# latticeboltzmann/2d-lb

Hardware: AMD Instinct MI355X
Metric: MLUPS (million lattice updates per second), fused D2Q9 BGK step (higher is better)
Workload: dtype f32

## Files before the change

2d-lb_amd/csrc/kernels_deep.h:

```cpp
#pragma once

#ifdef LB_DIAG
#define LB_DEEP_NOCOLLIDE if (!(a.diag & 1))
#else
#define LB_DEEP_NOCOLLIDE
#endif

namespace {

constexpr int DEEP_RW = 1, DEEP_PFD = 1;
constexpr int DEEP_WSLOTS = 8;
constexpr bool deep_pairs(bool mask, int bc) { return !mask && bc == LB_BC_PERIODIC; }

template <int RW, int NL>
struct DeepState {
    Window w[RW > 0 ? RW : 1];
    f4a d0[NL];
    unsigned mhist;
};
typedef unsigned u4v __attribute__((ext_vector_type(4)));
struct DeepCtx {
    int lane, x4, ym, n_iter;
    bool store_lane;
    f4a (*mine)[64], (*other)[64];
    f4a (*ho)[64];
    f4a (*dma)[64];
    unsigned dma_off;
};
constexpr int DEEP_WHOLE = 0, DEEP_FRONT = 1, DEEP_BACK = 2;
constexpr int DEEP_HO_SLOTS = 10;

__device__ __forceinline__ void deep_window_load(f4a (*W)[64], int lane, int it, f4a d0, Window &w)
{
    const int gs = 2 + 3 * (it & 1);
    w.d0 = d0; w.d1 = W[0][lane]; w.d3 = W[1][lane];
    w.g2 = W[gs][lane]; w.g5 = W[gs + 1][lane]; w.g6 = W[gs + 2][lane];
}
template <bool DOWN>
__device__ __forceinline__ void deep_window_push(f4a (*W)[64], int lane, int it, f4a &d0, const f4a (&q)[9])
{
    typedef Dir<DOWN> D_;
    const int gs = 2 + 3 * (it & 1);
    d0 = q[0]; W[0][lane] = q[1]; W[1][lane] = q[3];
    W[gs][lane] = q[D_::A]; W[gs + 1][lane] = q[D_::B]; W[gs + 2][lane] = q[D_::C];
}
template <bool DOWN>
__device__ __forceinline__ void deep_publish(f4a (*W)[64], int lane, int gs, const f4a (&q)[9])
{
    typedef Dir<DOWN> D_;
    W[gs][lane] = q[D_::An]; W[gs + 1][lane] = q[D_::Bn]; W[gs + 2][lane] = q[D_::Cn];
}

constexpr int DEEP_NUM_RECORDS = -1;
__device__ __forceinline__ float *deep_uniform(const float *p)
{
    const unsigned long long v = (unsigned long long)p;
    const unsigned lo = __builtin_amdgcn_readfirstlane((unsigned)v), hi = __builtin_amdgcn_readfirstlane((unsigned)(v >> 32));
    return reinterpret_cast<float *>(((unsigned long long)hi << 32) | lo);
}
__device__ __forceinline__ f4a deep_buf_load(__amdgpu_buffer_rsrc_t r, int vo, int so, int imm)
{
    return __builtin_bit_cast(f4a, __builtin_amdgcn_raw_buffer_load_b128(r, vo + imm, so, 0));
}
template <int BC, bool MASK>
__device__ __forceinline__ void deep_row_load(const StepArgs &a, int r, int x4, Row1 &o)
{
    int ym, yp;
    o.have = step1_rows(a, r, o.rr, ym, yp);
    o.mk = uc4{0, 0, 0, 0};
    o.hsolid = false;
    o.hxc = -1;
    if (o.have) {
        const long long P = a.pitch, S = a.plane;
        const float *s = a.src;
        const int yl = o.rr;
        o.wp = WrapPatch{0.f, 0.f, 0.f, 0.f, 0.f, 0.f};
        if (BC == LB_BC_PERIODIC) {
            const int c = a.nx - 1 - x4;
            const bool wrap_w = x4 == 0, wrap_e = c >= 0 && c < 4;
            if (wrap_w) {
                o.wp.p1 = s[1 * S + (long long)yl * P + a.nx - 1];
                o.wp.p5 = s[5 * S + (long long)ym * P + a.nx - 1];
                o.wp.p8 = s[8 * S + (long long)yp * P + a.nx - 1];
            }
            if (wrap_e) {
                o.wp.w3 = s[3 * S + (long long)yl * P];
                o.wp.w6 = s[6 * S + (long long)ym * P];
                o.wp.w7 = s[7 * S + (long long)yp * P];
            }
        }
        const __amdgpu_buffer_rsrc_t r0 = __builtin_amdgcn_make_buffer_rsrc(deep_uniform(s + (long long)yl * P - 1), 0, DEEP_NUM_RECORDS, 0x00020000);
        const __amdgpu_buffer_rsrc_t rm = __builtin_amdgcn_make_buffer_rsrc(deep_uniform(s + (long long)ym * P - 1), 0, DEEP_NUM_RECORDS, 0x00020000);
        const __amdgpu_buffer_rsrc_t rp = __builtin_amdgcn_make_buffer_rsrc(deep_uniform(s + (long long)yp * P - 1), 0, DEEP_NUM_RECORDS, 0x00020000);
        const unsigned S4 = (unsigned)a.plane * 4u;
        const int vo = x4 * 4;
        o.q[0] = deep_buf_load(r0, vo, 0, 4);
        o.q[1] = deep_buf_load(r0, vo, (int)(S4), 0);
        o.q[2] = deep_buf_load(rm, vo, (int)(2u * S4), 4);
        o.q[3] = deep_buf_load(r0, vo, (int)(3u * S4), 8);
        o.q[4] = deep_buf_load(rp, vo, (int)(4u * S4), 4);
        o.q[5] = deep_buf_load(rm, vo, (int)(5u * S4), 0);
        o.q[6] = deep_buf_load(rm, vo, (int)(6u * S4), 8);
        o.q[7] = deep_buf_load(rp, vo, (int)(7u * S4), 8);
        o.q[8] = deep_buf_load(rp, vo, (int)(8u * S4), 0);
        if (MASK) o.mk = *reinterpret_cast<const uc4 *>(lane_ptr(a.mask + (long long)yl * a.fpitch, x4));
    } else {
        o.wp = WrapPatch{0.f, 0.f, 0.f, 0.f, 0.f, 0.f};
#pragma unroll
        for (int k = 0; k < 9; ++k) o.q[k] = f4a{0.f, 0.f, 0.f, 0.f};
    }
}
#ifdef LB_DIAG
constexpr bool DEEP_MANUAL = false;
#else
constexpr bool DEEP_MANUAL = true;
#endif
__device__ __forceinline__ u4v deep_rsrc_words(const float *p)
{
    const unsigned long long v = (unsigned long long)p;
    return u4v{(unsigned)__builtin_amdgcn_readfirstlane((unsigned)v), (unsigned)__builtin_amdgcn_readfirstlane((unsigned)(v >> 32)), (unsigned)DEEP_NUM_RECORDS,
               0x00020000u};
}
template <int BC, bool MASK>
__device__ __forceinline__ void deep_row_issue(const StepArgs &a, int r, int x4, Row1 &o)
{
    int ym, yp;
    o.have = step1_rows(a, r, o.rr, ym, yp);
    o.hsolid = false;
    o.hxc = -1;
    if (o.have) {
        const long long P = a.pitch, S = a.plane;
        const float *s = a.src;
        const int yl = o.rr;
        if (BC == LB_BC_PERIODIC) {
            const int c = a.nx - 1 - x4;
            const bool wrap_w = x4 == 0, wrap_e = c >= 0 && c < 4;
            if (wrap_w) {
                const float *e = s + a.nx - 1;
                asm volatile("global_load_dword a36, %0, off\n\tglobal_load_dword a37, %1, off\n\tglobal_load_dword a38, %2, off"
                             :: "v"(e + 1 * S + (long long)yl * P), "v"(e + 5 * S + (long long)ym * P), "v"(e + 8 * S + (long long)yp * P)
                             : "memory", "a36", "a37", "a38");
            }
            if (wrap_e) {
                asm volatile("global_load_dword a39, %0, off\n\tglobal_load_dword a40, %1, off\n\tglobal_load_dword a41, %2, off"
                             :: "v"(s + 3 * S + (long long)yl * P), "v"(s + 6 * S + (long long)ym * P), "v"(s + 7 * S + (long long)yp * P)
                             : "memory", "a39", "a40", "a41");
            }
        }
        const u4v r0 = deep_rsrc_words(s + (long long)yl * P - 1), rm = deep_rsrc_words(s + (long long)ym * P - 1),
                  rp = deep_rsrc_words(s + (long long)yp * P - 1);
        const unsigned S4 = (unsigned)a.plane * 4u;
        asm volatile("buffer_load_dwordx4 a[0:3], %0, %1, 0 offen offset:4\n\t"
                     "buffer_load_dwordx4 a[4:7], %0, %1, %4 offen\n\t"
                     "buffer_load_dwordx4 a[8:11], %0, %2, %5 offen offset:4\n\t"
                     "buffer_load_dwordx4 a[12:15], %0, %1, %6 offen offset:8\n\t"
                     "buffer_load_dwordx4 a[16:19], %0, %3, %7 offen offset:4\n\t"
                     "buffer_load_dwordx4 a[20:23], %0, %2, %8 offen\n\t"
                     "buffer_load_dwordx4 a[24:27], %0, %2, %9 offen offset:8\n\t"
                     "buffer_load_dwordx4 a[28:31], %0, %3, %10 offen offset:8\n\t"
                     "buffer_load_dwordx4 a[32:35], %0, %3, %11 offen"
                     :: "v"(x4 * 4), "s"(r0), "s"(rm), "s"(rp), "s"(S4), "s"(2u * S4), "s"(3u * S4), "s"(4u * S4), "s"(5u * S4), "s"(6u * S4),
                        "s"(7u * S4), "s"(8u * S4)
                     : "memory", "a0", "a1", "a2", "a3", "a4", "a5", "a6", "a7", "a8", "a9", "a10", "a11", "a12", "a13",
                       "a14", "a15", "a16", "a17", "a18", "a19", "a20", "a21", "a22", "a23", "a24", "a25", "a26", "a27", "a28",
                       "a29", "a30", "a31", "a32", "a33", "a34", "a35");
        if (MASK) asm volatile("global_load_dword a42, %0, off" :: "v"(lane_ptr(a.mask + (long long)yl * a.fpitch, x4)) : "memory", "a42");
    }
}
template <int BC, bool MASK, int N>
__device__ __forceinline__ void deep_row_take(Row1 &o)
{
    static_assert(N == 0 || N == 9 || N == 12, "the stores of one steady iteration, or nothing");
#define LB_DEEP_TAKE_OUTS "={a[0:3]}"(o.q[0]), "={a[4:7]}"(o.q[1]), "={a[8:11]}"(o.q[2]), "={a[12:15]}"(o.q[3]), \
                          "={a[16:19]}"(o.q[4]), "={a[20:23]}"(o.q[5]), "={a[24:27]}"(o.q[6]), "={a[28:31]}"(o.q[7]), "={a[32:35]}"(o.q[8])
    if (N == 0) asm volatile("s_waitcnt vmcnt(0)" : LB_DEEP_TAKE_OUTS :: "memory");
    else if (N == 9) asm volatile("s_waitcnt vmcnt(9)" : LB_DEEP_TAKE_OUTS :: "memory");
    else asm volatile("s_waitcnt vmcnt(12)" : LB_DEEP_TAKE_OUTS :: "memory");
#undef LB_DEEP_TAKE_OUTS
    o.wp = WrapPatch{0.f, 0.f, 0.f, 0.f, 0.f, 0.f};
    if (BC == LB_BC_PERIODIC)
        asm volatile("" : "={a36}"(o.wp.p1), "={a37}"(o.wp.p5), "={a38}"(o.wp.p8), "={a39}"(o.wp.w3), "={a40}"(o.wp.w6), "={a41}"(o.wp.w7));
    o.mk = uc4{0, 0, 0, 0};
    if (MASK) {
        unsigned m;
        asm volatile("" : "={a42}"(m));
        o.mk = __builtin_bit_cast(uc4, m);
    }
    if (!o.have) {
#pragma unroll
        for (int k = 0; k < 9; ++k) o.q[k] = f4a{0.f, 0.f, 0.f, 0.f};
        o.mk = uc4{0, 0, 0, 0};
    }
}

template <int BC, bool MASK>
__device__ __forceinline__ void deep_row_issue_lds(const StepArgs &a, int r, int x4, unsigned slot, Row1 &o)
{
    int ym, yp;
    o.have = step1_rows(a, r, o.rr, ym, yp);
    o.hsolid = false;
    o.hxc = -1;
    if (o.have) {
        const long long P = a.pitch, S = a.plane;
        const float *s = a.src;
        const int yl = o.rr;
        unsigned m0_kept;
        asm volatile("s_waitcnt lgkmcnt(0)" ::: "memory");
        if (BC == LB_BC_PERIODIC) {
            const int c = a.nx - 1 - x4;
            const bool wrap_w = x4 == 0, wrap_e = c >= 0 && c < 4;
            if (wrap_w) {
                const float *e = s + a.nx - 1;
                asm volatile("s_mov_b32 %0, m0\n\ts_mov_b32 m0, %4\n\ts_nop 0\n\tglobal_load_lds_dword %1, off\n\t"
                             "s_add_u32 m0, m0, 0x100\n\ts_nop 0\n\tglobal_load_lds_dword %2, off\n\t"
                             "s_add_u32 m0, m0, 0x100\n\ts_nop 0\n\tglobal_load_lds_dword %3, off\n\ts_mov_b32 m0, %0"
                             : "=&s"(m0_kept)
                             : "v"(e + 1 * S + (long long)yl * P), "v"(e + 5 * S + (long long)ym * P), "v"(e + 8 * S + (long long)yp * P),
                               "s"(slot + 9 * 1024 + 256)
                             : "memory", "scc");
            }
            if (wrap_e) {
                asm volatile("s_mov_b32 %0, m0\n\ts_mov_b32 m0, %4\n\ts_nop 0\n\tglobal_load_lds_dword %1, off\n\t"
                             "s_add_u32 m0, m0, 0x100\n\ts_nop 0\n\tglobal_load_lds_dword %2, off\n\t"
                             "s_add_u32 m0, m0, 0x100\n\ts_nop 0\n\tglobal_load_lds_dword %3, off\n\ts_mov_b32 m0, %0"
                             : "=&s"(m0_kept)
                             : "v"(s + 3 * S + (long long)yl * P), "v"(s + 6 * S + (long long)ym * P), "v"(s + 7 * S + (long long)yp * P),
                               "s"(slot + 9 * 1024 + 256)
                             : "memory", "scc");
            }
        }
        const u4v r0 = deep_rsrc_words(s + (long long)yl * P - 1), rm = deep_rsrc_words(s + (long long)ym * P - 1),
                  rp = deep_rsrc_words(s + (long long)yp * P - 1);
        const unsigned S4 = (unsigned)a.plane * 4u;
        const int v0 = x4 * 4, v4 = v0 + 4, v8 = v0 + 8;
        asm volatile("s_mov_b32 %0, m0\n\ts_mov_b32 m0, %15\n\ts_nop 0\n\tbuffer_load_dwordx4 %2, %4, 0 offen lds\n\t"
                     "s_add_u32 m0, m0, 0x400\n\ts_nop 0\n\tbuffer_load_dwordx4 %1, %4, %7 offen lds\n\t"
                     "s_add_u32 m0, m0, 0x400\n\ts_nop 0\n\tbuffer_load_dwordx4 %2, %5, %8 offen lds\n\t"
                     "s_add_u32 m0, m0, 0x400\n\ts_nop 0\n\tbuffer_load_dwordx4 %3, %4, %9 offen lds\n\t"
                     "s_add_u32 m0, m0, 0x400\n\ts_nop 0\n\tbuffer_load_dwordx4 %2, %6, %10 offen lds\n\t"
                     "s_add_u32 m0, m0, 0x400\n\ts_nop 0\n\tbuffer_load_dwordx4 %1, %5, %11 offen lds\n\t"
                     "s_add_u32 m0, m0, 0x400\n\ts_nop 0\n\tbuffer_load_dwordx4 %3, %5, %12 offen lds\n\t"
                     "s_add_u32 m0, m0, 0x400\n\ts_nop 0\n\tbuffer_load_dwordx4 %3, %6, %13 offen lds\n\t"
                     "s_add_u32 m0, m0, 0x400\n\ts_nop 0\n\tbuffer_load_dwordx4 %1, %6, %14 offen lds\n\ts_mov_b32 m0, %0"
                     : "=&s"(m0_kept)
                     : "v"(v0), "v"(v4), "v"(v8), "s"(r0), "s"(rm), "s"(rp), "s"(S4), "s"(2u * S4), "s"(3u * S4), "s"(4u * S4), "s"(5u * S4),
                       "s"(6u * S4), "s"(7u * S4), "s"(8u * S4), "s"(slot)
                     : "memory", "scc");
        if (MASK)
            asm volatile("s_mov_b32 %0, m0\n\ts_mov_b32 m0, %2\n\ts_nop 0\n\tglobal_load_lds_dword %1, off\n\ts_mov_b32 m0, %0"
                         : "=&s"(m0_kept) : "v"(lane_ptr(a.mask + (long long)yl * a.fpitch, x4)), "s"(slot + 9 * 1024) : "memory");
    }
}
template <int BC, bool MASK>
__device__ __forceinline__ void deep_row_take_lds(const f4a (*S)[64], int lane, Row1 &o)
{
    asm volatile("s_waitcnt vmcnt(0)" ::: "memory");
    if (o.have) {
#pragma unroll
        for (int k = 0; k < 9; ++k) o.q[k] = S[k][lane];
        const unsigned *X = reinterpret_cast<const unsigned *>(S[9]);
        o.mk = MASK ? __builtin_bit_cast(uc4, X[lane]) : uc4{0, 0, 0, 0};
        o.wp = WrapPatch{0.f, 0.f, 0.f, 0.f, 0.f, 0.f};
        if (BC == LB_BC_PERIODIC) {
            const float e1 = __builtin_bit_cast(float, X[64 + lane]), e2 = __builtin_bit_cast(float, X[128 + lane]),
                        e3 = __builtin_bit_cast(float, X[192 + lane]);
            o.wp = WrapPatch{e1, e2, e3, e1, e2, e3};
        }
    } else {
        o.wp = WrapPatch{0.f, 0.f, 0.f, 0.f, 0.f, 0.f};
#pragma unroll
        for (int k = 0; k < 9; ++k) o.q[k] = f4a{0.f, 0.f, 0.f, 0.f};
        o.mk = uc4{0, 0, 0, 0};
    }
}

__device__ __forceinline__ void deep_row_store(const StepArgs &a, int r, int x4, const f4a (&t)[9])
{
    const __amdgpu_buffer_rsrc_t rd = __builtin_amdgcn_make_buffer_rsrc(deep_uniform(a.dst + (long long)r * a.pitch), 0, DEEP_NUM_RECORDS, 0x00020000);
    const unsigned S4 = (unsigned)a.plane * 4u;
    const int vo = x4 * 4;
    asm volatile("" ::: "memory");
    if (a.nts != 0) {
#pragma unroll
        for (int k = 0; k < 9; ++k) __builtin_amdgcn_raw_buffer_store_b128(__builtin_bit_cast(u4v, t[k]), rd, vo, (int)(k * S4), 2);
    } else {
#pragma unroll
        for (int k = 0; k < 9; ++k) __builtin_amdgcn_raw_buffer_store_b128(__builtin_bit_cast(u4v, t[k]), rd, vo, (int)(k * S4), 0);
    }
}

template <int BC, bool MASK, bool MACRO, int D, int RW, bool DOWN, int NST, int S, int ROLE = DEEP_WHOLE>
__device__ __forceinline__ void deep_stage(const StepArgs &a, const DeepCtx &cx, const int i, const int it,
                                           DeepState<RW, D - 1 - RW> &st, f4a (&qin)[9], f4a &r4, f4a &u4, f4a &v4)
{
    if constexpr (S <= D) {
        constexpr int K = S - 1;
        const int lane = cx.lane, x4 = cx.x4;
        constexpr int L = K > RW ? K - RW - 1 : 0;
        f4a (*W)[64] = cx.mine + L * DEEP_WSLOTS;
        if constexpr (NST >= S) {
            int r, t0_, t1_;
            (void)step1_rows(a, DOWN ? cx.ym - 1 - (i - K) : cx.ym + (i - K), r, t0_, t1_);
            f4a t[9];
            if constexpr (K <= RW) {
                skirt_gather<DOWN>(st.w[K - 1], qin, t);
                window_push_dir<DOWN>(st.w[K - 1], qin);
            } else {
                Window w;
                deep_window_load(W, lane, it, st.d0[L], w);
                skirt_gather<DOWN>(w, qin, t);
                deep_window_push<DOWN>(W, lane, it, st.d0[L], qin);
            }
            LB_DEEP_NOCOLLIDE collide_row<BC, MASK, true>(a, x4, a.y0 + r, t, mask_bits(st.mhist, K), r4, u4, v4);
            if constexpr (S == D && ROLE == DEEP_FRONT) {
#pragma unroll
                for (int k = 0; k < 9; ++k) cx.ho[k][lane] = t[k];
                if (MASK) reinterpret_cast<unsigned *>(cx.ho[9])[lane] = __builtin_bit_cast(unsigned, mask_bits(st.mhist, K));
            } else if constexpr (S == D) {
#ifdef LB_DIAG
                if (!(a.diag & (1 << 22)))
#endif
                if (cx.store_lane) {
                    deep_row_store(a, r, x4, t);
                    if (MACRO) {
                        const long long m = (long long)r * a.fpitch;
                        store_moments(a, m, x4, r4, u4, v4);
                    }
                }
            } else {
                if constexpr (NST == S) {
                    if constexpr (S <= RW) deep_publish<DOWN>(cx.other + (D - 2 - RW) * DEEP_WSLOTS, lane, S == 1 ? 5 : 2, t);
                    else deep_publish<DOWN>(cx.other + (S - RW - 1) * DEEP_WSLOTS, lane, 2 + 3 * (S & 1), t);
                }
                deep_stage<BC, MASK, MACRO, D, RW, DOWN, NST, S + 1, ROLE>(a, cx, i, it, st, t, r4, u4, v4);
            }
        } else if constexpr (NST == S - 1) {
            if constexpr (K <= RW) window_push_dir<DOWN>(st.w[K - 1], qin);
            else deep_window_push<DOWN>(W, lane, it, st.d0[L], qin);
        }
    }
}

template <int BC, bool MASK, bool MACRO, int D, int RW, int PFD, bool DOWN, int NST, int PAR = -1, int ROLE = DEEP_WHOLE>
__device__ __forceinline__ void deep_iter(const StepArgs &a, const DeepCtx &cx, const int i_, DeepState<RW, D - 1 - RW> &st, Row1 &cur,
                                          Row1 &nxt)
{
    static_assert(RW >= 0 && RW <= 2 && D - 1 - RW >= 1 && (ROLE == DEEP_WHOLE ? D - 2 > RW : D - 2 >= RW),
                  "register windows hand over through the last LDS window while it is idle");
    static_assert((D - 1 - RW) * DEEP_WSLOTS <= 40, "a wave has 40 KB of LDS at four waves per CU");
    const int lane = cx.lane, x4 = cx.x4;
    const int i = NST < D ? NST - 1 : i_;
    const int it = PAR >= 0 ? PAR : i;
    auto row_at = [&](int p) { return DOWN ? cx.ym - 1 - p : cx.ym + p; };
    f4a (*MB)[64] = cx.mine + (D - 2 - RW) * DEEP_WSLOTS;
    if (RW >= 1 && NST == 2) { st.w[0].g2 = MB[5][lane]; st.w[0].g5 = MB[6][lane]; st.w[0].g6 = MB[7][lane]; }
    if (RW >= 2 && NST == 3) { st.w[RW >= 2 ? 1 : 0].g2 = MB[2][lane]; st.w[RW >= 2 ? 1 : 0].g5 = MB[3][lane]; st.w[RW >= 2 ? 1 : 0].g6 = MB[4][lane]; }
#ifdef LB_DIAG
    if (!((a.diag & (1 << 23)) && i > 0))
#endif
    if constexpr (ROLE != DEEP_BACK) {
        if (ROLE == DEEP_FRONT) {
            deep_row_take_lds<BC, MASK>(cx.dma, lane, cur);
            deep_row_issue_lds<BC, MASK>(a, row_at(min(i + 1, cx.n_iter - 1)), x4, cx.dma_off, nxt);
        } else if (PFD && DEEP_MANUAL) {
            deep_row_take<BC, MASK, (NST < D ? 0 : (MACRO ? 12 : 9))>(cur);
            deep_row_issue<BC, MASK>(a, row_at(min(i + 1, cx.n_iter - 1)), x4, nxt);
        } else {
            static_assert(PFD == 1 || ROLE == DEEP_BACK, "a march that gathers its rows gathers them one ahead");
            deep_row_load<BC, MASK>(a, row_at(min(i + 1, cx.n_iter - 1)), x4, nxt);
        }
    }
    f4a (&q1)[9] = cur.q;
    f4a r4, u4, v4;
    const uc4 mk = cur.mk;
    if (ROLE != DEEP_BACK && cur.have) {
        gather_merge<BC, true>(a, x4, q1, cur.wp);
        LB_DEEP_NOCOLLIDE collide_row<BC, MASK, true>(a, x4, a.y0 + cur.rr, q1, mk, r4, u4, v4);
    }
    if (NST == 1) {
        if constexpr (RW >= 1) deep_publish<DOWN>(cx.other + (D - 2 - RW) * DEEP_WSLOTS, lane, 5, q1);
        else deep_publish<DOWN>(cx.other, lane, 2 + 3 * 1, q1);
    }
    deep_stage<BC, MASK, MACRO, D, RW, DOWN, NST, 2, ROLE>(a, cx, i, it, st, q1, r4, u4, v4);
    if (MASK) st.mhist = ((st.mhist | mask_word(mk)) << 1) & (0x01010101u * (unsigned)(((1 << D) - 2) & 0xff));
    if (ROLE == DEEP_WHOLE && NST < D) __syncthreads();
}

template <int BC, bool MASK, bool MACRO, int D, int RW, int PFD, bool DOWN, int NST>
__device__ __forceinline__ void deep_fill(const StepArgs &a, const DeepCtx &cx, DeepState<RW, D - 1 - RW> &st, Row1 &ra, Row1 &rb)
{
    if constexpr (NST < D) {
        if ((NST & 1) == 0) deep_iter<BC, MASK, MACRO, D, RW, PFD, DOWN, NST>(a, cx, NST - 1, st, rb, ra);
        else deep_iter<BC, MASK, MACRO, D, RW, PFD, DOWN, NST>(a, cx, NST - 1, st, ra, rb);
        deep_fill<BC, MASK, MACRO, D, RW, PFD, DOWN, NST + 1>(a, cx, st, ra, rb);
    }
}

template <int BC, bool MASK, bool MACRO, int D, int RW, int PFD, bool DOWN>
__device__ __forceinline__ void deep_march(const StepArgs &a, const int x0, const int ym, const int len, f4a (*mine)[64],
                                           f4a (*other)[64])
{
    DeepCtx cx;
    cx.lane = threadIdx.x;
    const int xr = x0 + cx.lane * 4;
    cx.x4 = skirt_column<BC>(a, xr, deep_skirt_lanes(D));
    cx.store_lane = skirt_store_lane(a, cx.lane, xr, deep_skirt_lanes(D));
    cx.ym = ym; cx.n_iter = len + D - 1;
    cx.mine = mine; cx.other = other;
    DeepState<RW, D - 1 - RW> st = {};
    auto row_at = [&](int p) { return DOWN ? ym - 1 - p : ym + p; };
    static_assert(PFD == 1, "a whole march gathers one row ahead");
    Row1 ra, rb;
    if (DEEP_MANUAL) deep_row_issue<BC, MASK>(a, row_at(0), cx.x4, ra);
    else deep_row_load<BC, MASK>(a, row_at(0), cx.x4, ra);
    deep_fill<BC, MASK, MACRO, D, RW, PFD, DOWN, 1>(a, cx, st, ra, rb);
    if (DEEP_MANUAL) asm volatile("s_waitcnt vmcnt(0)" ::: "memory");
    if (!deep_pairs(MASK, BC)) {
        if ((D - 1) & 1) ra = rb;
        for (int i = D - 1; i < cx.n_iter; ++i) {
            deep_iter<BC, MASK, MACRO, D, RW, PFD, DOWN, D>(a, cx, i, st, ra, rb);
            ra = rb;
        }
    } else {
        constexpr int P0 = (D - 1) & 1;
        int i = D - 1;
        for (; i + 1 < cx.n_iter; i += 2) {
            deep_iter<BC, MASK, MACRO, D, RW, PFD, DOWN, D, P0>(a, cx, i, st, P0 ? rb : ra, P0 ? ra : rb);
            deep_iter<BC, MASK, MACRO, D, RW, PFD, DOWN, D, 1 - P0>(a, cx, i + 1, st, P0 ? ra : rb, P0 ? rb : ra);
        }
        if (i < cx.n_iter) deep_iter<BC, MASK, MACRO, D, RW, PFD, DOWN, D, P0>(a, cx, i, st, P0 ? rb : ra, P0 ? ra : rb);
    }
    if (DEEP_MANUAL) asm volatile("s_waitcnt vmcnt(0)" ::: "memory");
}

template <int BC, bool MASK, bool MACRO, int D, int RW, int PFD>
__global__ __launch_bounds__(64 * STEP4_WAVES, PFD ? 1 : 2) void k_deep(const StepArgs a, int strips, int seg_rows, int nsegs, int row_end)
{
    __shared__ f4a lds_win[STEP4_WAVES][(D - 1 - RW) * DEEP_WSLOTS][64];
    const int wy = __builtin_amdgcn_readfirstlane(threadIdx.y);
    const int item = xcd_item(blockIdx.x, gridDim.x);
#ifdef LB_DIAG
    const unsigned long long diag_t0 = __builtin_amdgcn_s_memrealtime();
#endif
    int sx, sy;
    if (item < strips * nsegs) {
        sx = item % strips;
        sy = item / strips;
    } else {
        if (!a.edge_seg_rows) return;
        const int j = item - strips * nsegs;
        sx = (j & 1) ? strips - 1 : 0;
        sy = nsegs + (j >> 1);
    }
    int stride = a.seg_stride;
    if (a.edge_seg_rows && (sx == 0 || sx == strips - 1)) stride = seg_rows = a.edge_seg_rows;
    const int ya = a.row_begin + sy * stride;
    if (ya >= row_end) return;
    const int yb = min(ya + seg_rows, row_end);
    const int ym = ya + (yb - ya) / 2;
    const int x0 = sx * deep_valid(D) - 4 * deep_skirt_lanes(D);
    if (wy == 0) deep_march<BC, MASK, MACRO, D, RW, PFD, true>(a, x0, ym, ym - ya, lds_win[0], lds_win[1]);
    else deep_march<BC, MASK, MACRO, D, RW, PFD, false>(a, x0, ym, yb - ym, lds_win[1], lds_win[0]);
#ifdef LB_DIAG
    if ((a.diag & 4096) && threadIdx.x == 0) {
        __builtin_amdgcn_s_waitcnt(0);
        const unsigned long long t1 = __builtin_amdgcn_s_memrealtime();
        unsigned *o = reinterpret_cast<unsigned *>(a.rho) + 8 * (item * STEP4_WAVES + wy);
        o[0] = (unsigned)diag_t0; o[1] = (unsigned)(diag_t0 >> 32); o[2] = (unsigned)t1; o[3] = (unsigned)(t1 >> 32);
        o[4] = __builtin_amdgcn_s_getreg((31 << 11) | 20);
        o[5] = __builtin_amdgcn_s_getreg((31 << 11) | 4);
        o[6] = (unsigned)(item * STEP4_WAVES + wy); o[7] = (unsigned)(wy ? yb - ym : ym - ya);
    }
#endif
}

}
```

2d-lb_amd/csrc/kernels_deep2.h:

```cpp
#pragma once

namespace {

constexpr int deep2_split(int D) { return D >= 8 ? 4 : (D + 1) / 2; }
constexpr int deep2_rw_front(int D) { return deep2_split(D) - 2 >= 2 ? 2 : 1; }
constexpr int deep2_rw_back(int D) { return (D - deep2_split(D) + 1) - 2 >= 2 ? 2 : 1; }
constexpr int DEEP2_WAVES = 4;

__device__ __forceinline__ void deep2_barrier() { asm volatile("s_waitcnt lgkmcnt(0)\n\ts_barrier" ::: "memory"); }

template <int BC, bool MASK, int F, int RW, bool DOWN, int NST>
__device__ __forceinline__ void deep2_front_fill(const StepArgs &a, const DeepCtx &cx, DeepState<RW, F - 1 - RW> &st, Row1 &ra, Row1 &rb,
                                                 int &trip)
{
    if constexpr (NST < F) {
        deep2_barrier();
        if (trip < cx.n_iter) {
            if ((NST & 1) == 0) deep_iter<BC, MASK, false, F, RW, 1, DOWN, NST, -1, DEEP_FRONT>(a, cx, NST - 1, st, rb, ra);
            else deep_iter<BC, MASK, false, F, RW, 1, DOWN, NST, -1, DEEP_FRONT>(a, cx, NST - 1, st, ra, rb);
        }
        deep2_barrier();
        ++trip;
        deep2_front_fill<BC, MASK, F, RW, DOWN, NST + 1>(a, cx, st, ra, rb, trip);
    }
}

template <int BC, bool MASK, int D, int F, int RW, bool DOWN>
__device__ __forceinline__ void deep2_front(const StepArgs &a, const int x0, const int ym, const int len, const int trips, f4a (*mine)[64],
                                            f4a (*other)[64], f4a (*ho)[64], f4a (*dma)[64])
{
    DeepCtx cx;
    cx.lane = threadIdx.x;
    const int xr = x0 + cx.lane * 4;
    cx.x4 = skirt_column<BC>(a, xr, deep_skirt_lanes(D));
    cx.store_lane = false;
    cx.ym = ym; cx.n_iter = len + D - 1;
    cx.mine = mine; cx.other = other; cx.ho = ho; cx.dma = dma;
    cx.dma_off = __builtin_amdgcn_readfirstlane((unsigned)reinterpret_cast<unsigned long long>(dma));
    DeepState<RW, F - 1 - RW> st = {};
    auto row_at = [&](int p) { return DOWN ? ym - 1 - p : ym + p; };
    Row1 ra, rb;
    deep_row_issue_lds<BC, MASK>(a, row_at(0), cx.x4, cx.dma_off, ra);
    int trip = 0;
    deep2_front_fill<BC, MASK, F, RW, DOWN, 1>(a, cx, st, ra, rb, trip);
    if ((F - 1) & 1) ra = rb;
    for (; trip < trips; ++trip) {
#ifdef LB_DIAG
        if (!(a.diag & (1 << 24)))
#endif
        deep2_barrier();
        if (trip < cx.n_iter) {
            deep_iter<BC, MASK, false, F, RW, 1, DOWN, F, -1, DEEP_FRONT>(a, cx, trip, st, ra, rb);
            ra = rb;
        }
#ifdef LB_DIAG
        if (!(a.diag & (1 << 24)))
#endif
        deep2_barrier();
    }
    asm volatile("s_waitcnt vmcnt(0)" ::: "memory");
}

template <bool MASK>
__device__ __forceinline__ void deep2_take(const DeepCtx &cx, Row1 &cur)
{
#pragma unroll
    for (int k = 0; k < 9; ++k) cur.q[k] = cx.ho[k][cx.lane];
    cur.mk = uc4{0, 0, 0, 0};
    if (MASK) cur.mk = __builtin_bit_cast(uc4, reinterpret_cast<const unsigned *>(cx.ho[9])[cx.lane]);
    cur.have = true;
}

template <int BC, bool MASK, bool MACRO, int DB, int RW, bool DOWN, int NST>
__device__ __forceinline__ void deep2_back_fill(const StepArgs &a, const DeepCtx &cx, DeepState<RW, DB - 1 - RW> &st, Row1 &cur, int &j)
{
    if constexpr (NST < DB) {
        if (j < cx.n_iter) deep2_take<MASK>(cx, cur);
        deep2_barrier();
        if (j < cx.n_iter) deep_iter<BC, MASK, MACRO, DB, RW, 0, DOWN, NST, -1, DEEP_BACK>(a, cx, NST - 1, st, cur, cur);
        deep2_barrier();
        ++j;
        deep2_back_fill<BC, MASK, MACRO, DB, RW, DOWN, NST + 1>(a, cx, st, cur, j);
    }
}

template <int BC, bool MASK, bool MACRO, int D, int F, int RW, bool DOWN>
__device__ __forceinline__ void deep2_back(const StepArgs &a, const int x0, const int ym, const int len, const int trips, f4a (*mine)[64],
                                           f4a (*other)[64], f4a (*ho)[64])
{
    constexpr int DB = D - F + 1;
    DeepCtx cx;
    cx.lane = threadIdx.x;
    const int xr = x0 + cx.lane * 4;
    cx.x4 = skirt_column<BC>(a, xr, deep_skirt_lanes(D));
    cx.store_lane = skirt_store_lane(a, cx.lane, xr, deep_skirt_lanes(D));
    cx.ym = ym; cx.n_iter = len + DB - 1;
    cx.mine = mine; cx.other = other; cx.ho = ho;
    DeepState<RW, DB - 1 - RW> st = {};
    Row1 cur;
    cur.wp = WrapPatch{0.f, 0.f, 0.f, 0.f, 0.f, 0.f};
    cur.hsolid = false; cur.hxc = -1; cur.rr = 0;
    for (int t = 0; t < F; ++t) {
        deep2_barrier();
        deep2_barrier();
    }
    int j = 0;
    deep2_back_fill<BC, MASK, MACRO, DB, RW, DOWN, 1>(a, cx, st, cur, j);
    for (; j + F < trips; ++j) {
        if (j < cx.n_iter) deep2_take<MASK>(cx, cur);
#ifdef LB_DIAG
        if (!(a.diag & (1 << 24)))
#endif
        deep2_barrier();
        if (j < cx.n_iter) deep_iter<BC, MASK, MACRO, DB, RW, 0, DOWN, DB, -1, DEEP_BACK>(a, cx, j, st, cur, cur);
#ifdef LB_DIAG
        if (!(a.diag & (1 << 24)))
#endif
        deep2_barrier();
    }
}

template <int BC, bool MASK, bool MACRO, int D>
__global__ __launch_bounds__(64 * DEEP2_WAVES, 2) void k_deep2(const StepArgs a, int strips, int seg_rows, int nsegs, int row_end)
{
    constexpr int F = deep2_split(D), RWF = deep2_rw_front(D), RWB = deep2_rw_back(D);
    constexpr int LF = (F - 1 - RWF) * DEEP_WSLOTS, LBK = (D - F - RWB) * DEEP_WSLOTS;
    static_assert(2 * (LF + LBK + 2 * DEEP_HO_SLOTS) <= 80, "two workgroups per CU: 80 KB each");
    __shared__ f4a lds_dma[2][DEEP_HO_SLOTS][64];
    __shared__ f4a lds_front[2][LF][64];
    __shared__ f4a lds_back[2][LBK][64];
    __shared__ f4a lds_ho[2][DEEP_HO_SLOTS][64];
    const int wy = (__builtin_amdgcn_readfirstlane(threadIdx.y) + ((blockIdx.x >> 8) & 1) * 2) & 3;
    const int item = xcd_item(blockIdx.x, gridDim.x);
#ifdef LB_DIAG
    const unsigned long long diag_t0 = __builtin_amdgcn_s_memrealtime();
#endif
    int sx, sy;
    if (item < strips * nsegs) {
        sx = item % strips;
        sy = item / strips;
    } else {
        if (!a.edge_seg_rows) return;
        const int j = item - strips * nsegs;
        sx = (j & 1) ? strips - 1 : 0;
        sy = nsegs + (j >> 1);
    }
    int stride = a.seg_stride;
    if (a.edge_seg_rows && (sx == 0 || sx == strips - 1)) stride = seg_rows = a.edge_seg_rows;
    const int ya = a.row_begin + sy * stride;
    if (ya >= row_end) return;
    const int yb = min(ya + seg_rows, row_end);
    const int ym = ya + (yb - ya) / 2;
    const int x0 = sx * deep_valid(D) - 4 * deep_skirt_lanes(D);
    const int trips = max(ym - ya, yb - ym) + D;
    if (wy == 0) deep2_front<BC, MASK, D, F, RWF, true>(a, x0, ym, ym - ya, trips, lds_front[0], lds_front[1], lds_ho[0], lds_dma[0]);
    else if (wy == 1) deep2_front<BC, MASK, D, F, RWF, false>(a, x0, ym, yb - ym, trips, lds_front[1], lds_front[0], lds_ho[1], lds_dma[1]);
    else if (wy == 2) deep2_back<BC, MASK, MACRO, D, F, RWB, true>(a, x0, ym, ym - ya, trips, lds_back[0], lds_back[1], lds_ho[0]);
    else deep2_back<BC, MASK, MACRO, D, F, RWB, false>(a, x0, ym, yb - ym, trips, lds_back[1], lds_back[0], lds_ho[1]);
#ifdef LB_DIAG
    if ((a.diag & 4096) && threadIdx.x == 0) {
        __builtin_amdgcn_s_waitcnt(0);
        const unsigned long long t1 = __builtin_amdgcn_s_memrealtime();
        unsigned *o = reinterpret_cast<unsigned *>(a.rho) + 8 * (item * DEEP2_WAVES + wy);
        o[0] = (unsigned)diag_t0; o[1] = (unsigned)(diag_t0 >> 32); o[2] = (unsigned)t1; o[3] = (unsigned)(t1 >> 32);
        o[4] = __builtin_amdgcn_s_getreg((31 << 11) | 20);
        o[5] = __builtin_amdgcn_s_getreg((31 << 11) | 4);
        o[6] = (unsigned)(item * DEEP2_WAVES + wy); o[7] = (unsigned)((wy & 1) ? yb - ym : ym - ya);
    }
#endif
}

}
```

2d-lb_amd/csrc/kernels_fused.h:

```cpp
#pragma once
#include <type_traits>
#include "d2q9_cell.h"
#include "plan_consts.h"

struct StepArgs {
    const float *src;
    float *dst;
    const uint8_t *mask;
    float *rho, *u, *v;
    long long plane;
    int pitch;
    int fpitch;
    int nx, ny;
    int y0, h;
    int row_begin, row_step, row_count;
    int wrap_y;
    int ghost_s, ghost_n;
    int seg_stride;
    int edge_seg_rows;
    int diag;
    int prio_turns;
    int nts;
    int tile_launch_order;
    float omega, rho_in, rho_out, lid_u, rho0;
    float u_w, u_e;
    const float *corner;
};

constexpr int BATCH_MAX = 8;
struct BatchArgs {
    StepArgs a[BATCH_MAX];
};

namespace {

template <int BC>
__device__ __forceinline__ void boundary_rule(const StepArgs &a, Cell &c, bool w, bool e, bool s, bool n)
{
    if (BC == LB_BC_PIPE) bc_pipe_cell(c, w, e, s, n, a.rho_in, a.rho_out);
    if (BC == LB_BC_PIPE_I) bc_pipe_i_cell(c, w, e, s, n, a.rho_in, a.rho_out);
    if (BC == LB_BC_CAVITY) bc_cavity_cell(c, w, e, s, n, a.lid_u, a.rho0);
    if (BC == LB_BC_VELOCITY_INLET && (w || e)) bc_vel_cell(c, w, e, s, n, a.u_w, a.u_e, a.corner);
}

template <int BC>
__device__ __noinline__ Cell boundary_rule_call(Cell c, int wesn, float p0, float p1)
{
    const bool w = wesn & 1, e = wesn & 2, s = wesn & 4, n = wesn & 8;
    if (BC == LB_BC_PIPE) bc_pipe_cell(c, w, e, s, n, p0, p1);
    if (BC == LB_BC_PIPE_I) bc_pipe_i_cell(c, w, e, s, n, p0, p1);
    if (BC == LB_BC_CAVITY) bc_cavity_cell(c, w, e, s, n, p0, p1);
    return c;
}

template <int BC, bool MASK>
__device__ __forceinline__ void finish_cell(const StepArgs &a, int x, int yl, Cell &c, bool solid, float &rho, float &ux,
                                            float &uy)
{
    if (MASK) bounce_cell(c, solid);
    if (BC == LB_BC_VELOCITY_INLET) {
        moments_cell(c, rho, ux, uy);
        if (x == 0 || x == a.nx - 1) {
            const long long o = (long long)yl * a.fpitch + x;
            const int yg = a.y0 + yl;
            vel_moments_cell(c, x == 0, yg == 0, yg == a.ny - 1, a.u_w, a.u_e, a.u[o], a.v[o], rho, ux, uy);
        }
        equilibrate_cell(c, a.omega, rho, ux, uy);
    } else if (BC == LB_BC_PIPE_I) {
        moments_i_cell(c, rho, ux, uy);
        if (MASK && solid) { ux = 0.f; uy = 0.f; }
        equilibrate_i_cell(c, a.omega, rho, ux, uy);
    } else {
        relax_cell(c, a.omega, rho, ux, uy);
    }
}

template <typename T>
__device__ __forceinline__ T *lane_ptr(T *row, int x)
{
    typedef typename std::conditional<std::is_const<T>::value, const char, char>::type B;
    return reinterpret_cast<T *>(reinterpret_cast<B *>(row) + (unsigned)x * (unsigned)sizeof(T));
}

struct WrapPatch {
    float p1, p5, p8, w3, w6, w7;
};

template <int BC, bool MASK, bool NTL>
__device__ __forceinline__ void gather_issue(const StepArgs &a, int x4, int yl, int ym, int yp, f4a (&q)[9], uc4 &mk,
                                             WrapPatch &wp)
{
    const long long P = a.pitch, S = a.plane;
    const float *s = a.src;
    const float *r0 = s + (long long)yl * P, *rm = s + (long long)ym * P, *rp = s + (long long)yp * P;
    wp = WrapPatch{0.f, 0.f, 0.f, 0.f, 0.f, 0.f};
#ifdef LB_DIAG
    if (a.diag & 8) {
        q[0] = load4<NTL>(lane_ptr(r0, x4));          q[1] = load4<NTL>(lane_ptr(r0 + 1 * S, x4));
        q[2] = load4<NTL>(lane_ptr(rm + 2 * S, x4));  q[3] = load4<NTL>(lane_ptr(r0 + 3 * S, x4));
        q[4] = load4<NTL>(lane_ptr(rp + 4 * S, x4));  q[5] = load4<NTL>(lane_ptr(rm + 5 * S, x4));
        q[6] = load4<NTL>(lane_ptr(rm + 6 * S, x4));  q[7] = load4<NTL>(lane_ptr(rp + 7 * S, x4));
        q[8] = load4<NTL>(lane_ptr(rp + 8 * S, x4));
        mk = uc4{0, 0, 0, 0};
        return;
    }
#endif
    if (BC == LB_BC_PERIODIC) {
        const int c = a.nx - 1 - x4;
        bool wrap_w = x4 == 0, wrap_e = c >= 0 && c < 4;
#ifdef LB_DIAG
        if (a.diag & 16384) wrap_w = wrap_e = false;
#endif
        if (wrap_w) {
            wp.p1 = s[1 * S + (long long)yl * P + a.nx - 1];
            wp.p5 = s[5 * S + (long long)ym * P + a.nx - 1];
            wp.p8 = s[8 * S + (long long)yp * P + a.nx - 1];
        }
        if (wrap_e) {
            wp.w3 = s[3 * S + (long long)yl * P];
            wp.w6 = s[6 * S + (long long)ym * P];
            wp.w7 = s[7 * S + (long long)yp * P];
        }
    }
    q[0] = load4<NTL>(lane_ptr(r0, x4));
    q[1] = load4u<NTL>(lane_ptr(r0 + 1 * S - 1, x4));
    q[2] = load4<NTL>(lane_ptr(rm + 2 * S, x4));
    q[3] = load4u<NTL>(lane_ptr(r0 + 3 * S + 1, x4));
    q[4] = load4<NTL>(lane_ptr(rp + 4 * S, x4));
    q[5] = load4u<NTL>(lane_ptr(rm + 5 * S - 1, x4));
    q[6] = load4u<NTL>(lane_ptr(rm + 6 * S + 1, x4));
    q[7] = load4u<NTL>(lane_ptr(rp + 7 * S + 1, x4));
    q[8] = load4u<NTL>(lane_ptr(rp + 8 * S - 1, x4));
    mk = uc4{0, 0, 0, 0};
    if (MASK) mk = *reinterpret_cast<const uc4 *>(lane_ptr(a.mask + (long long)yl * a.fpitch, x4));
}

template <int BC, bool ALIGNED4 = false>
__device__ __forceinline__ void gather_merge(const StepArgs &a, int x4, f4a (&q)[9], const WrapPatch &wp)
{
    if (BC == LB_BC_PERIODIC && ALIGNED4) {
        bool wrap_w = x4 == 0, wrap_e = x4 == a.nx - 4;
#ifdef LB_DIAG
        if (a.diag & (8 | 16384)) wrap_w = wrap_e = false;
#endif
        q[1].x = wrap_w ? wp.p1 : q[1].x;
        q[5].x = wrap_w ? wp.p5 : q[5].x;
        q[8].x = wrap_w ? wp.p8 : q[8].x;
        q[3].w = wrap_e ? wp.w3 : q[3].w;
        q[6].w = wrap_e ? wp.w6 : q[6].w;
        q[7].w = wrap_e ? wp.w7 : q[7].w;
    } else if (BC == LB_BC_PERIODIC) {
        const int c = a.nx - 1 - x4;
        bool wrap_w = x4 == 0, wrap_e = c >= 0 && c < 4;
#ifdef LB_DIAG
        if (a.diag & (8 | 16384)) wrap_w = wrap_e = false;
#endif
        q[1].x = wrap_w ? wp.p1 : q[1].x;
        q[5].x = wrap_w ? wp.p5 : q[5].x;
        q[8].x = wrap_w ? wp.p8 : q[8].x;
#pragma unroll
        for (int j = 0; j < 4; ++j) {
            const bool hit = wrap_e && j == c;
            q[3][j] = hit ? wp.w3 : q[3][j];
            q[6][j] = hit ? wp.w6 : q[6][j];
            q[7][j] = hit ? wp.w7 : q[7][j];
        }
    }
}

template <int BC, bool MASK, bool NTL>
__device__ __forceinline__ void gather_row(const StepArgs &a, int x4, int yl, int ym, int yp, f4a (&q)[9], uc4 &mk)
{
    WrapPatch wp;
    gather_issue<BC, MASK, NTL>(a, x4, yl, ym, yp, q, mk, wp);
    gather_merge<BC>(a, x4, q, wp);
}

__device__ __forceinline__ void store_row9(bool nts, float *d, long long S, int x4, const f4a (&t)[9])
{
    const int kS = (int)S;
    if (nts) {
        asm volatile("" : "+v"(x4) : : "memory");
#pragma unroll
        for (int k = 0; k < 9; ++k) store4<true>(lane_ptr(d, x4 + k * kS), t[k]);
        asm volatile("" ::: "memory");
    } else {
        asm volatile("" : "+v"(x4));
#pragma unroll
        for (int k = 0; k < 9; ++k) store4<false>(lane_ptr(d, x4 + k * kS), t[k]);
    }
}

__device__ __forceinline__ void store_moments(const StepArgs &a, long long m, int x4, f4a r4, f4a u4, f4a v4)
{
    store4<false>(lane_ptr(a.rho + m, x4), r4);
    store4<false>(lane_ptr(a.u + m, x4), u4);
    store4<false>(lane_ptr(a.v + m, x4), v4);
}

__device__ __forceinline__ Cell row_cell(const f4a (&q)[9], int j)
{
    return Cell{q[0][j], q[1][j], q[2][j], q[3][j], q[4][j], q[5][j], q[6][j], q[7][j], q[8][j]};
}
__device__ __forceinline__ void row_cell_put(f4a (&q)[9], int j, const Cell &c)
{
    q[0][j] = c.f0; q[1][j] = c.f1; q[2][j] = c.f2; q[3][j] = c.f3; q[4][j] = c.f4;
    q[5][j] = c.f5; q[6][j] = c.f6; q[7][j] = c.f7; q[8][j] = c.f8;
}

template <int BC, bool MASK, bool OOL = false>
__device__ __forceinline__ void collide_row(const StepArgs &a, int x4, int yg, f4a (&q)[9], uc4 mk, f4a &r4,
                                            f4a &u4, f4a &v4)
{
    if (BC != LB_BC_PERIODIC) {
        const bool south = (yg == 0), north = (yg == a.ny - 1);
        bool wall_row = (BC != LB_BC_VELOCITY_INLET) && (south || north);
        bool first = (x4 == 0);
        bool last = (x4 <= a.nx - 1 && a.nx - 1 < x4 + 4);
        const int jl = (a.nx - 1) & 3;
#ifdef LB_DIAG
        if (a.diag & 512) wall_row = first = last = false;
#endif
        if (wall_row || first || last) {
#pragma unroll
            for (int j = 0; j < 4; ++j) {
                if (wall_row || (first && j == 0) || (last && j == jl)) {
                    Cell c = row_cell(q, j);
                    const bool w = first && j == 0, e = last && j == jl;
                    if constexpr (OOL && (BC == LB_BC_PIPE || BC == LB_BC_PIPE_I || BC == LB_BC_CAVITY)) {
                        const bool cav = (BC == LB_BC_CAVITY);
                        c = boundary_rule_call<BC>(c, (w ? 1 : 0) | (e ? 2 : 0) | (south ? 4 : 0) | (north ? 8 : 0),
                                                   cav ? a.lid_u : a.rho_in, cav ? a.rho0 : a.rho_out);
                    } else {
                        boundary_rule<BC>(a, c, w, e, south, north);
                    }
                    row_cell_put(q, j, c);
                }
            }
        }
    }
    if (BC == LB_BC_VELOCITY_INLET) {
        Cell c[4];
        float rho[4], ux[4], uy[4];
#pragma unroll
        for (int j = 0; j < 4; ++j) {
            c[j] = row_cell(q, j);
            if (MASK) bounce_cell(c[j], mk[j] != 0);
            moments_cell(c[j], rho[j], ux[j], uy[j]);
        }
        const bool first = (x4 == 0), last = (x4 <= a.nx - 1 && a.nx - 1 < x4 + 4);
        if (first || last) {
            const int jl = (a.nx - 1) & 3;
#pragma unroll
            for (int j = 0; j < 4; ++j)
                if ((first && j == 0) || (last && j == jl)) {
                    const long long o = (long long)(yg - a.y0) * a.fpitch + x4 + j;
                    vel_moments_cell(c[j], first && j == 0, yg == 0, yg == a.ny - 1, a.u_w, a.u_e, a.u[o], a.v[o], rho[j], ux[j],
                                     uy[j]);
                }
        }
#pragma unroll
        for (int j = 0; j < 4; ++j) {
            equilibrate_cell(c[j], a.omega, rho[j], ux[j], uy[j]);
            r4[j] = rho[j]; u4[j] = ux[j]; v4[j] = uy[j];
            row_cell_put(q, j, c[j]);
        }
        return;
    }
    if (BC == LB_BC_PIPE_I) {
#pragma unroll
        for (int j = 0; j < 4; ++j) {
            Cell c = row_cell(q, j);
            float rho, ux, uy;
            finish_cell<BC, MASK>(a, x4 + j, yg - a.y0, c, mk[j] != 0, rho, ux, uy);
            r4[j] = rho; u4[j] = ux; v4[j] = uy;
            row_cell_put(q, j, c);
        }
        return;
    }
#pragma unroll
    for (int h = 0; h < 2; ++h) {
        f2a f[9];
#pragma unroll
        for (int k = 0; k < 9; ++k) f[k] = h ? q[k].zw : q[k].xy;
        if (MASK) {
            const bool s0 = mk[2 * h] != 0, s1 = mk[2 * h + 1] != 0;
            auto swap2 = [&](f2a &p, f2a &o) {
                const f2a pp = p, oo = o;
                p = f2a{s0 ? oo.x : pp.x, s1 ? oo.y : pp.y};
                o = f2a{s0 ? pp.x : oo.x, s1 ? pp.y : oo.y};
            };
            swap2(f[1], f[3]); swap2(f[2], f[4]); swap2(f[5], f[7]); swap2(f[6], f[8]);
        }
        f2a rho, ux, uy;
        moments_t<f2a>(f[0], f[1], f[2], f[3], f[4], f[5], f[6], f[7], f[8], rho, ux, uy);
        equilibrate_t<f2a>(f[0], f[1], f[2], f[3], f[4], f[5], f[6], f[7], f[8], a.omega, rho, ux, uy);
        if (h) { r4.zw = rho; u4.zw = ux; v4.zw = uy; }
        else   { r4.xy = rho; u4.xy = ux; v4.xy = uy; }
#pragma unroll
        for (int k = 0; k < 9; ++k) {
            if (h) q[k].zw = f[k];
            else q[k].xy = f[k];
        }
    }
}

template <int BC, bool MASK, bool MACRO, bool NTL, bool NTS, bool XCD>
__device__ __forceinline__ void step_body(const StepArgs &a)
{
    int bx = blockIdx.x, by = blockIdx.y;
    if (XCD) {
        const unsigned total = gridDim.x * gridDim.y;
        const unsigned lin = blockIdx.y * gridDim.x + blockIdx.x;
        const unsigned per = total >> 3;
        if (lin < (per << 3)) {
            const unsigned t = (lin & 7u) * per + (lin >> 3);
            bx = t % gridDim.x;
            by = t / gridDim.x;
        }
    }
    const int x4 = (bx * blockDim.x + threadIdx.x) * 4;
    const int ri = by * blockDim.y + __builtin_amdgcn_readfirstlane(threadIdx.y);
    if (x4 >= a.fpitch || ri >= a.row_count) return;
    const int yl = a.row_begin + ri * a.row_step;
    const int yg = a.y0 + yl;
    int ym = yl - 1, yp = yl + 1;
    if (a.wrap_y == 1) {
        if (ym < 0) ym = a.h - 1;
        if (yp >= a.h) yp = 0;
    } else if (a.wrap_y == 2) {
        if (ym < 0) ym = a.h - 2;
        if (yp >= a.h) yp = 1;
    }
    const long long o0 = (long long)yl * a.pitch;
    f4a q[9], r4, u4, v4;
    uc4 mk;
    gather_row<BC, MASK, NTL>(a, x4, yl, ym, yp, q, mk);
#ifdef LB_DIAG
    if (!(a.diag & 1))
#endif
    collide_row<BC, MASK>(a, x4, yg, q, mk, r4, u4, v4);

    const long long S = a.plane;
    float *d = a.dst + o0;
#pragma unroll
    for (int k = 0; k < 9; ++k) store4<NTS>(lane_ptr(d + k * S, x4), q[k]);
    if (MACRO) {
        const long long m0 = (long long)yl * a.fpitch;
        store_moments(a, m0, x4, r4, u4, v4);
    }
}

template <int BC, bool MASK, bool MACRO, bool NTL, bool NTS, bool XCD>
__global__ __launch_bounds__(256) void k_step(const StepArgs a)
{
    step_body<BC, MASK, MACRO, NTL, NTS, XCD>(a);
}

template <int BC, bool MASK, bool MACRO>
__global__ __launch_bounds__(256) void k_step_batch(const BatchArgs b)
{
    step_body<BC, MASK, MACRO, false, false, false>(b.a[blockIdx.z]);
}


__device__ __forceinline__ int xcd_item(int wg, int nwg)
{
    const int blk = wg & ~63, i = wg & 63;
    return (blk + 64 <= nwg) ? blk + (i & 7) * 8 + (i >> 3) : wg;
}

__device__ __forceinline__ f4a from_left(f4a v, float halo, int lane)
{
    float w = __shfl_up(v.w, 1);
    if (lane == 0) w = halo;
    return f4a{w, v.x, v.y, v.z};
}
__device__ __forceinline__ f4a from_right(f4a v, float halo, int lane)
{
    float x = __shfl_down(v.x, 1);
    if (lane == 63) x = halo;
    return f4a{v.y, v.z, v.w, x};
}

__device__ __forceinline__ bool step1_rows(const StepArgs &a, int r, int &rr, int &ym, int &yp)
{
    const int h = a.h, w = a.wrap_y, per = h - (w == 2 ? 1 : 0);
    const int wr = r < 0 ? r + per : (r >= h ? r - per : r);
    rr = w ? wr : r;
    const int m = rr - 1, p = rr + 1;
    ym = (w && m < 0) ? h - w : m;
    yp = (w && p >= h) ? w - 1 : p;
    return w || (r < 0 ? a.ghost_s != 0 : (r >= h ? a.ghost_n != 0 : true));
}

template <int BC, bool MASK>
__device__ __forceinline__ void halo_cell_load(const StepArgs &a, int hx, int rr, int ym, int yp, Cell &c, bool &solid,
                                               int &xc)
{
    solid = false;
    xc = hx;
    int xl = hx - 1, xg = hx + 1;
    if (BC == LB_BC_PERIODIC) {
        xc = hx < 0 ? hx + a.nx : (hx >= a.nx ? hx - a.nx : hx);
        xl = xc - 1 < 0 ? a.nx - 1 : xc - 1;
        xg = xc + 1 >= a.nx ? 0 : xc + 1;
    } else if (hx < 0 || hx >= a.nx) {
        c = Cell{0.f, 0.f, 0.f, 0.f, 0.f, 0.f, 0.f, 0.f, 0.f};
        xc = -1;
        return;
    }
    const long long P = a.pitch, S = a.plane;
    const float *s = a.src;
    const float *r0 = s + (long long)rr * P, *rm = s + (long long)ym * P, *rp = s + (long long)yp * P;
    c.f0 = *lane_ptr(r0, xc);
    c.f1 = *lane_ptr(r0 + 1 * S, xl);
    c.f2 = *lane_ptr(rm + 2 * S, xc);
    c.f3 = *lane_ptr(r0 + 3 * S, xg);
    c.f4 = *lane_ptr(rp + 4 * S, xc);
    c.f5 = *lane_ptr(rm + 5 * S, xl);
    c.f6 = *lane_ptr(rm + 6 * S, xg);
    c.f7 = *lane_ptr(rp + 7 * S, xg);
    c.f8 = *lane_ptr(rp + 8 * S, xl);
    if (MASK) solid = *lane_ptr(a.mask + (long long)rr * a.fpitch, xc) != 0;
}

template <int BC, bool MASK>
__device__ __forceinline__ void halo_cell_finish(const StepArgs &a, int xc, int rr, Cell &c, bool solid)
{
    if (BC != LB_BC_PERIODIC && xc < 0) return;
    const int yg = a.y0 + rr;
    if (BC != LB_BC_PERIODIC && (yg == 0 || yg == a.ny - 1 || xc == 0 || xc == a.nx - 1))
        boundary_rule<BC>(a, c, xc == 0, xc == a.nx - 1, yg == 0, yg == a.ny - 1);
    float rho, ux, uy;
    finish_cell<BC, MASK>(a, xc, rr, c, solid, rho, ux, uy);
}

template <int BC, bool MASK>
__device__ __forceinline__ void halo_cell_step1(const StepArgs &a, int hx, int rr, int ym, int yp, Cell &c,
                                                bool &solid)
{
    int xc;
    halo_cell_load<BC, MASK>(a, hx, rr, ym, yp, c, solid, xc);
    halo_cell_finish<BC, MASK>(a, xc, rr, c, solid);
}

template <int BC, bool MASK, bool MACRO>
__global__ __launch_bounds__(256, 2) void k_step2(const StepArgs a, int strips, int seg_rows, int nsegs, int row_end)
{
    const int lane = threadIdx.x;
    const int item = xcd_item(blockIdx.x, gridDim.x) * 4 + __builtin_amdgcn_readfirstlane(threadIdx.y);
    const int sx = item % strips, sy = item / strips;
    if (sy >= nsegs) return;
    const int ya = a.row_begin + sy * a.seg_stride;
    if (ya >= row_end) return;
    const int yb = min(ya + seg_rows, row_end);
    const int x0 = sx * STRIP_W;
    const int xr = x0 + lane * 4;
    int x4 = xr;
    if (BC == LB_BC_PERIODIC && xr >= a.nx) x4 = xr - a.nx;
    const bool store_lane = xr < a.nx;
    const bool edge_lane = (lane == 0) || (lane == 63);
    const int hx = (lane == 0) ? x0 - 1 : x0 + STRIP_W;
    const long long S = a.plane;

    f4a d0 = {}, d1 = {}, d3 = {};
    f4a e2 = {}, e5 = {}, e6 = {};
    f4a g2 = {}, g5 = {}, g6 = {};
    float hd = 0.f, he = 0.f, hg = 0.f;
    uc4 mk_prev = {0, 0, 0, 0};
    for (int r = ya - 1; r <= yb; ++r) {
        f4a q[9], r4, u4, v4;
        uc4 mk = {0, 0, 0, 0};
        int rr, ym, yp;
        const bool have = step1_rows(a, r, rr, ym, yp);
        float hq0 = 0.f, hq1 = 0.f, hq2 = 0.f;
        if (have) {
            gather_row<BC, MASK, false>(a, x4, rr, ym, yp, q, mk);
            if (edge_lane) {
                Cell hc;
                bool hsolid;
                halo_cell_step1<BC, MASK>(a, hx, rr, ym, yp, hc, hsolid);
                hq0 = lane == 0 ? hc.f1 : hc.f3;
                hq1 = lane == 0 ? hc.f5 : hc.f6;
                hq2 = lane == 0 ? hc.f8 : hc.f7;
            }
#ifdef LB_DIAG
            if (!(a.diag & 1))
#endif
            collide_row<BC, MASK>(a, x4, a.y0 + rr, q, mk, r4, u4, v4);
        } else {
#pragma unroll
            for (int k = 0; k < 9; ++k) q[k] = f4a{0.f, 0.f, 0.f, 0.f};
        }
        if (r >= ya + 1) {
            const int y = r - 1;
            f4a t[9];
            t[0] = d0;
            t[1] = from_left(d1, hd, lane);
            t[3] = from_right(d3, hd, lane);
            t[2] = g2;
            t[5] = from_left(g5, hg, lane);
            t[6] = from_right(g6, hg, lane);
            t[4] = q[4];
            t[7] = from_right(q[7], hq2, lane);
            t[8] = from_left(q[8], hq2, lane);
            const long long o = (long long)y * a.pitch;
#ifdef LB_DIAG
            if (!(a.diag & 2))
#endif
            collide_row<BC, MASK>(a, x4, a.y0 + y, t, mk_prev, r4, u4, v4);
#ifdef LB_DIAG
            if (a.diag & 4) {
#pragma unroll
                for (int k = 0; k < 9; ++k) asm volatile("" ::"v"(t[k]));
            } else
#endif
            if (store_lane) {
                float *d = a.dst + o;
                store_row9(a.nts != 0, d, S, x4, t);
                if (MACRO) {
                    const long long m = (long long)y * a.fpitch;
                    store_moments(a, m, x4, r4, u4, v4);
                }
            }
        }
        g2 = e2; g5 = e5; g6 = e6;
        e2 = q[2]; e5 = q[5]; e6 = q[6];
        d0 = q[0]; d1 = q[1]; d3 = q[3];
        hg = he; he = hq1; hd = hq0;
        mk_prev = mk;
    }
}


struct HaloLinks {
    float c0, c2, c4;
    float t0, tp, tm;
};

__device__ __forceinline__ HaloLinks halo_links(const Cell &c, bool left)
{
    HaloLinks h;
    h.c0 = c.f0; h.c2 = c.f2; h.c4 = c.f4;
    h.t0 = left ? c.f1 : c.f3;
    h.tp = left ? c.f5 : c.f6;
    h.tm = left ? c.f8 : c.f7;
    return h;
}

struct Window {
    f4a d0, d1, d3;
    f4a e2, e5, e6;
    f4a g2, g5, g6;
};
__device__ __forceinline__ void window_push(Window &w, const f4a (&q)[9])
{
    w.g2 = w.e2; w.g5 = w.e5; w.g6 = w.e6;
    w.e2 = q[2]; w.e5 = q[5]; w.e6 = q[6];
    w.d0 = q[0]; w.d1 = q[1]; w.d3 = q[3];
}
struct HaloWindow {
    float t0_d, tp_e, tp_g;
    float c0_d, c2_e, c2_g;
};
__device__ __forceinline__ void halo_push(HaloWindow &w, const HaloLinks &h)
{
    w.tp_g = w.tp_e; w.tp_e = h.tp; w.t0_d = h.t0;
    w.c2_g = w.c2_e; w.c2_e = h.c2; w.c0_d = h.c0;
}

__device__ __forceinline__ void window_gather(const Window &w, const f4a (&q)[9], const HaloWindow &hw,
                                              const HaloLinks &hnew, int lane, f4a (&t)[9])
{
    t[0] = w.d0;
    t[1] = from_left(w.d1, hw.t0_d, lane);
    t[3] = from_right(w.d3, hw.t0_d, lane);
    t[2] = w.g2;
    t[5] = from_left(w.g5, hw.tp_g, lane);
    t[6] = from_right(w.g6, hw.tp_g, lane);
    t[4] = q[4];
    t[7] = from_right(q[7], hnew.tm, lane);
    t[8] = from_left(q[8], hnew.tm, lane);
}

__device__ __forceinline__ unsigned mask_word(uc4 m)
{
    return (m.x ? 1u : 0u) | (m.y ? 0x100u : 0u) | (m.z ? 0x10000u : 0u) | (m.w ? 0x1000000u : 0u);
}
__device__ __forceinline__ uc4 mask_bits(unsigned hist, int age)
{
    const unsigned b = (hist >> age) & 0x01010101u;
    return uc4{(unsigned char)(b & 0xff), (unsigned char)((b >> 8) & 0xff), (unsigned char)((b >> 16) & 0xff),
               (unsigned char)(b >> 24)};
}

template <int BC, bool MASK, bool MACRO>
__global__ __launch_bounds__(256, 2) void k_step3(const StepArgs a, int strips, int seg_rows, int nsegs, int row_end)
{
    const int lane = threadIdx.x;
    const int item = xcd_item(blockIdx.x, gridDim.x) * 4 + __builtin_amdgcn_readfirstlane(threadIdx.y);
    const int sx = item % strips, sy = item / strips;
    if (sy >= nsegs) return;
    const int ya = a.row_begin + sy * a.seg_stride;
    if (ya >= row_end) return;
    const int yb = min(ya + seg_rows, row_end);
    const int x0 = sx * STRIP_W;
    const int xr = x0 + lane * 4;
    int x4 = xr;
    if (BC == LB_BC_PERIODIC && xr >= a.nx) x4 = xr - a.nx;
    const bool store_lane = xr < a.nx;
    const bool left = (lane == 0);
    const bool edge_lane = left || (lane == 63);
    const int hxi = left ? x0 - 1 : x0 + STRIP_W;
    const int hxo = left ? x0 - 2 : x0 + STRIP_W + 1;
    int hxi_c = hxi;
    if (BC == LB_BC_PERIODIC) hxi_c = hxi < 0 ? hxi + a.nx : (hxi >= a.nx ? hxi - a.nx : hxi);
    const bool hxi_in = (BC == LB_BC_PERIODIC) || (hxi >= 0 && hxi < a.nx);
    const long long S = a.plane;

    Window w1 = {}, w2 = {};
    HaloWindow hi1 = {}, ho1 = {}, hi2 = {};
    unsigned mhist = 0;
    for (int r = ya - 2; r <= yb + 1; ++r) {
        f4a q1[9], r4, u4, v4;
        uc4 mk = {0, 0, 0, 0};
        int rr, ym, yp;
        const bool have = step1_rows(a, r, rr, ym, yp);
        HaloLinks hi_new = {}, ho_new = {};
        bool hsolid = false;
        if (have) {
            gather_row<BC, MASK, false>(a, x4, rr, ym, yp, q1, mk);
            if (edge_lane) {
                Cell c;
                bool osolid;
                halo_cell_step1<BC, MASK>(a, hxi, rr, ym, yp, c, hsolid);
                hi_new = halo_links(c, left);
                halo_cell_step1<BC, MASK>(a, hxo, rr, ym, yp, c, osolid);
                ho_new = halo_links(c, left);
            }
#ifdef LB_DIAG
            if (!(a.diag & 1))
#endif
            collide_row<BC, MASK>(a, x4, a.y0 + rr, q1, mk, r4, u4, v4);
        } else {
#pragma unroll
            for (int k = 0; k < 9; ++k) q1[k] = f4a{0.f, 0.f, 0.f, 0.f};
        }
        f4a q2[9];
        HaloLinks h2_new = {};
        if (r >= ya) {
            int r2, r2m, r2p;
            (void)step1_rows(a, r - 1, r2, r2m, r2p);
            window_gather(w1, q1, hi1, hi_new, lane, q2);
            if (edge_lane) {
                Cell c;
                c.f0 = hi1.c0_d; c.f2 = hi1.c2_g; c.f4 = hi_new.c4;
                const float a0 = ho1.t0_d, ap = ho1.tp_g, am = ho_new.tm;
                const float b0 = left ? w1.d3.x : w1.d1.w;
                const float bp = left ? w1.g6.x : w1.g5.w;
                const float bm = left ? q1[7].x : q1[8].w;
                c.f1 = left ? a0 : b0; c.f3 = left ? b0 : a0;
                c.f5 = left ? ap : bp; c.f6 = left ? bp : ap;
                c.f8 = left ? am : bm; c.f7 = left ? bm : am;
                if (hxi_in) {
                    const int yg = a.y0 + r2;
                    if (BC != LB_BC_PERIODIC && (yg == 0 || yg == a.ny - 1 || hxi_c == 0 || hxi_c == a.nx - 1))
                        boundary_rule<BC>(a, c, hxi_c == 0, hxi_c == a.nx - 1, yg == 0, yg == a.ny - 1);
                    float rho, ux, uy;
                    finish_cell<BC, MASK>(a, hxi_c, r2, c, (mhist & 0x40u) != 0, rho, ux, uy);
                }
                h2_new = halo_links(c, left);
            }
#ifdef LB_DIAG
            if (!(a.diag & 2))
#endif
            collide_row<BC, MASK>(a, x4, a.y0 + r2, q2, mask_bits(mhist, 1), r4, u4, v4);
        } else {
#pragma unroll
            for (int k = 0; k < 9; ++k) q2[k] = f4a{0.f, 0.f, 0.f, 0.f};
        }
        if (r >= ya + 2) {
            int r3, r3m, r3p;
            (void)step1_rows(a, r - 2, r3, r3m, r3p);
            f4a t[9];
            window_gather(w2, q2, hi2, h2_new, lane, t);
            const long long o = (long long)r3 * a.pitch;
#ifdef LB_DIAG
            if (!(a.diag & 4))
#endif
            collide_row<BC, MASK>(a, x4, a.y0 + r3, t, mask_bits(mhist, 2), r4, u4, v4);
            if (store_lane) {
                float *d = a.dst + o;
                store_row9(a.nts != 0, d, S, x4, t);
                if (MACRO) {
                    const long long m = (long long)r3 * a.fpitch;
                    store_moments(a, m, x4, r4, u4, v4);
                }
            }
        }
        window_push(w1, q1);
        window_push(w2, q2);
        halo_push(hi1, hi_new);
        halo_push(ho1, ho_new);
        halo_push(hi2, h2_new);
        if (MASK) mhist = ((mhist | mask_word(mk) | (hsolid ? 0x20u : 0u)) << 1) & 0x06060646u;
    }
}

template <bool NT>
__global__ __launch_bounds__(256) void k_copy4(const f4a *__restrict__ src, f4a *__restrict__ dst, long long n4)
{
    const long long i = (long long)blockIdx.x * blockDim.x + threadIdx.x;
    if (i >= n4) return;
    if (NT) __builtin_nontemporal_store(__builtin_nontemporal_load(src + i), dst + i);
    else dst[i] = src[i];
}

}
```

Baseline: 485,600.

## March rows with incremental uniform cursors and hoist seam loads out of hot path

Replaces per-row recomputation of wrapped row indices and 64-bit source/destination addresses with a row cursor that advances lag/mid/lead byte offsets incrementally and keeps them wave-uniform in scalar registers. Periodic seam (wrap-column) loads and merges move into separate functions that run only for waves holding a boundary lane, chosen by a ballot, so interior waves skip that branch and its address arithmetic. This aims to cut scalar/vector integer overhead in the streaming loop. The trade-off is extra cursor state held in registers and more complex bookkeeping for the ghost/wrap cases.

```diff
diff --git a/2d-lb_amd/csrc/kernels_deep.h b/2d-lb_amd/csrc/kernels_deep.h
--- a/2d-lb_amd/csrc/kernels_deep.h
+++ b/2d-lb_amd/csrc/kernels_deep.h
@@ -115,40 +115,73 @@
 #else
 constexpr bool DEEP_MANUAL = true;
 #endif
-__device__ __forceinline__ u4v deep_rsrc_words(const float *p)
-{
-    const unsigned long long v = (unsigned long long)p;
-    return u4v{(unsigned)__builtin_amdgcn_readfirstlane((unsigned)v), (unsigned)__builtin_amdgcn_readfirstlane((unsigned)(v >> 32)), (unsigned)DEEP_NUM_RECORDS,
-               0x00020000u};
-}
-template <int BC, bool MASK>
-__device__ __forceinline__ void deep_row_issue(const StepArgs &a, int r, int x4, Row1 &o)
-{
-    int ym, yp;
-    o.have = step1_rows(a, r, o.rr, ym, yp);
+struct DeepRows {
+    RowMarch m;
+    RowCursor g;
+    RowTrack st;
+    int seam;
+    int flight;
+};
+__device__ __forceinline__ int deep_flight(const DeepRows &R) { return R.g.have ? R.m.h : 0; }
+__device__ __forceinline__ long long deep_uniform_ll(long long v)
+{
+    const unsigned lo = __builtin_amdgcn_readfirstlane((unsigned)v), hi = __builtin_amdgcn_readfirstlane((unsigned)((unsigned long long)v >> 32));
+    return (long long)(((unsigned long long)hi << 32) | lo);
+}
+template <int BC, bool DOWN>
+__device__ __forceinline__ DeepRows deep_rows_begin(const StepArgs &a, int r0, int x4)
+{
+    DeepRows R;
+    R.m = row_march(a.h, BC == LB_BC_PERIODIC ? a.wrap_y : 0, a.ghost_s, a.ghost_n, 4u * (unsigned)a.pitch);
+    R.g = row_cursor_begin<!DOWN>(R.m, r0, (long long)reinterpret_cast<unsigned long long>(a.src - 1));
+    R.g.mid.o = deep_uniform_ll(R.g.mid.o); R.g.lag = deep_uniform_ll(R.g.lag); R.g.lead = deep_uniform_ll(R.g.lead);
+    R.st = RowTrack{R.g.mid.y, deep_uniform_ll((long long)reinterpret_cast<unsigned long long>(a.dst) + (long long)R.g.mid.y * (long long)R.m.pitch_b)};
+    R.flight = 0;
+    R.seam = BC == LB_BC_PERIODIC && __builtin_amdgcn_ballot_w64(x4 == 0 || x4 == a.nx - 4) != 0 ? 1 : 0;
+    return R;
+}
+__device__ __forceinline__ u4v deep_rsrc_words(long long base)
+{
+    return u4v{(unsigned)base, (unsigned)((unsigned long long)base >> 32), (unsigned)DEEP_NUM_RECORDS, 0x00020000u};
+}
+__device__ __forceinline__ const float *deep_row_ptr(long long base) { return reinterpret_cast<const float *>((unsigned long long)base); }
+template <bool DOWN>
+__device__ __forceinline__ void deep_seam_issue(const StepArgs &a, const DeepRows &R, int x4)
+{
+    if (R.g.have) {
+        const long long S = a.plane;
+        const long long b0 = R.g.mid.o, bm = row_cursor_ym<!DOWN>(R.g), bp = row_cursor_yp<!DOWN>(R.g);
+        const bool wrap_w = x4 == 0, wrap_e = x4 == a.nx - 4;
+        if (wrap_w) {
+            const float *e0 = deep_row_ptr(b0) + a.nx, *em = deep_row_ptr(bm) + a.nx, *ep = deep_row_ptr(bp) + a.nx;
+            asm volatile("global_load_dword a36, %0, off\n\tglobal_load_dword a37, %1, off\n\tglobal_load_dword a38, %2, off"
+                         :: "v"(e0 + 1 * S), "v"(em + 5 * S), "v"(ep + 8 * S)
+                         : "memory", "a36", "a37", "a38");
+        }
+        if (wrap_e) {
+            asm volatile("global_load_dword a39, %0, off\n\tglobal_load_dword a40, %1, off\n\tglobal_load_dword a41, %2, off"
+                         :: "v"(deep_row_ptr(b0) + 1 + 3 * S), "v"(deep_row_ptr(bm) + 1 + 6 * S), "v"(deep_row_ptr(bp) + 1 + 7 * S)
+                         : "memory", "a39", "a40", "a41");
+        }
+    }
+}
+__device__ __forceinline__ void deep_seam_take(const StepArgs &a, int have, int x4, Row1 &o)
+{
+    asm volatile("" : "={a36}"(o.wp.p1), "={a37}"(o.wp.p5), "={a38}"(o.wp.p8), "={a39}"(o.wp.w3), "={a40}"(o.wp.w6), "={a41}"(o.wp.w7));
+    if (have) gather_merge<LB_BC_PERIODIC, true>(a, x4, o.q, o.wp);
+}
+template <int BC, bool MASK, bool DOWN>
+__device__ __forceinline__ void deep_row_issue(const StepArgs &a, DeepRows &R, int x4, Row1 &o)
+{
+    R.flight = deep_flight(R);
+    o.have = R.g.have != 0;
+    o.rr = R.g.rr();
     o.hsolid = false;
     o.hxc = -1;
-    if (o.have) {
-        const long long P = a.pitch, S = a.plane;
-        const float *s = a.src;
+    if (__builtin_expect(R.g.have != 0, 1)) {
         const int yl = o.rr;
-        if (BC == LB_BC_PERIODIC) {
-            const int c = a.nx - 1 - x4;
-            const bool wrap_w = x4 == 0, wrap_e = c >= 0 && c < 4;
-            if (wrap_w) {
-                const float *e = s + a.nx - 1;
-                asm volatile("global_load_dword a36, %0, off\n\tglobal_load_dword a37, %1, off\n\tglobal_load_dword a38, %2, off"
-                             :: "v"(e + 1 * S + (long long)yl * P), "v"(e + 5 * S + (long long)ym * P), "v"(e + 8 * S + (long long)yp * P)
-                             : "memory", "a36", "a37", "a38");
-            }
-            if (wrap_e) {
-                asm volatile("global_load_dword a39, %0, off\n\tglobal_load_dword a40, %1, off\n\tglobal_load_dword a41, %2, off"
-                             :: "v"(s + 3 * S + (long long)yl * P), "v"(s + 6 * S + (long long)ym * P), "v"(s + 7 * S + (long long)yp * P)
-                             : "memory", "a39", "a40", "a41");
-            }
-        }
-        const u4v r0 = deep_rsrc_words(s + (long long)yl * P - 1), rm = deep_rsrc_words(s + (long long)ym * P - 1),
-                  rp = deep_rsrc_words(s + (long long)yp * P - 1);
+        const long long b0 = R.g.mid.o, bm = row_cursor_ym<!DOWN>(R.g), bp = row_cursor_yp<!DOWN>(R.g);
+        const u4v r0 = deep_rsrc_words(b0), rm = deep_rsrc_words(bm), rp = deep_rsrc_words(bp);
         const unsigned S4 = (unsigned)a.plane * 4u;
         asm volatile("buffer_load_dwordx4 a[0:3], %0, %1, 0 offen offset:4\n\t"
                      "buffer_load_dwordx4 a[4:7], %0, %1, %4 offen\n\t"
@@ -178,59 +211,73 @@
     else asm volatile("s_waitcnt vmcnt(12)" : LB_DEEP_TAKE_OUTS :: "memory");
 #undef LB_DEEP_TAKE_OUTS
     o.wp = WrapPatch{0.f, 0.f, 0.f, 0.f, 0.f, 0.f};
-    if (BC == LB_BC_PERIODIC)
-        asm volatile("" : "={a36}"(o.wp.p1), "={a37}"(o.wp.p5), "={a38}"(o.wp.p8), "={a39}"(o.wp.w3), "={a40}"(o.wp.w6), "={a41}"(o.wp.w7));
     o.mk = uc4{0, 0, 0, 0};
     if (MASK) {
         unsigned m;
         asm volatile("" : "={a42}"(m));
         o.mk = __builtin_bit_cast(uc4, m);
     }
-    if (!o.have) {
-#pragma unroll
-        for (int k = 0; k < 9; ++k) o.q[k] = f4a{0.f, 0.f, 0.f, 0.f};
-        o.mk = uc4{0, 0, 0, 0};
-    }
-}
-
-template <int BC, bool MASK>
-__device__ __forceinline__ void deep_row_issue_lds(const StepArgs &a, int r, int x4, unsigned slot, Row1 &o)
-{
-    int ym, yp;
-    o.have = step1_rows(a, r, o.rr, ym, yp);
+}
+__device__ __forceinline__ void deep_row_none(Row1 &o)
+{
+#pragma unroll
+    for (int k = 0; k < 9; ++k) o.q[k] = f4a{0.f, 0.f, 0.f, 0.f};
+    o.mk = uc4{0, 0, 0, 0};
+}
+
+template <bool DOWN>
+__device__ __forceinline__ void deep_seam_issue_lds(const StepArgs &a, const DeepRows &R, int x4, unsigned slot)
+{
+    if (R.g.have) {
+        const long long S = a.plane;
+        const long long b0 = R.g.mid.o, bm = row_cursor_ym<!DOWN>(R.g), bp = row_cursor_yp<!DOWN>(R.g);
+        unsigned m0_kept;
+        asm volatile("s_waitcnt lgkmcnt(0)" ::: "memory");
+        const bool wrap_w = x4 == 0, wrap_e = x4 == a.nx - 4;
+        if (wrap_w) {
+            const float *e0 = deep_row_ptr(b0) + a.nx, *em = deep_row_ptr(bm) + a.nx, *ep = deep_row_ptr(bp) + a.nx;
+            asm volatile("s_mov_b32 %0, m0\n\ts_mov_b32 m0, %4\n\ts_nop 0\n\tglobal_load_lds_dword %1, off\n\t"
+                         "s_add_u32 m0, m0, 0x100\n\ts_nop 0\n\tglobal_load_lds_dword %2, off\n\t"
+                         "s_add_u32 m0, m0, 0x100\n\ts_nop 0\n\tglobal_load_lds_dword %3, off\n\ts_mov_b32 m0, %0"
+                         : "=&s"(m0_kept)
+                         : "v"(e0 + 1 * S), "v"(em + 5 * S), "v"(ep + 8 * S), "s"(slot + 9 * 1024 + 256)
+                         : "memory", "scc");
+        }
+        if (wrap_e) {
+            asm volatile("s_mov_b32 %0, m0\n\ts_mov_b32 m0, %4\n\ts_nop 0\n\tglobal_load_lds_dword %1, off\n\t"
+                         "s_add_u32 m0, m0, 0x100\n\ts_nop 0\n\tglobal_load_lds_dword %2, off\n\t"
+                         "s_add_u32 m0, m0, 0x100\n\ts_nop 0\n\tglobal_load_lds_dword %3, off\n\ts_mov_b32 m0, %0"
+                         : "=&s"(m0_kept)
+                         : "v"(deep_row_ptr(b0) + 1 + 3 * S), "v"(deep_row_ptr(bm) + 1 + 6 * S), "v"(deep_row_ptr(bp) + 1 + 7 * S),
+                           "s"(slot + 9 * 1024 + 256)
+                         : "memory", "scc");
+        }
+    }
+}
+__device__ __forceinline__ void deep_seam_take_lds(const StepArgs &a, int have, int x4, const f4a (*S)[64], int lane, Row1 &o)
+{
+    if (have) {
+        const unsigned *X = reinterpret_cast<const unsigned *>(S[9]);
+        const float e1 = __builtin_bit_cast(float, X[64 + lane]), e2 = __builtin_bit_cast(float, X[128 + lane]),
+                    e3 = __builtin_bit_cast(float, X[192 + lane]);
+        o.wp = WrapPatch{e1, e2, e3, e1, e2, e3};
+        gather_merge<LB_BC_PERIODIC, true>(a, x4, o.q, o.wp);
+    }
+}
+template <int BC, bool MASK, bool DOWN>
+__device__ __forceinline__ void deep_row_issue_lds(const StepArgs &a, DeepRows &R, int x4, unsigned slot, Row1 &o)
+{
+    R.flight = deep_flight(R);
+    o.have = R.g.have != 0;
+    o.rr = R.g.rr();
     o.hsolid = false;
     o.hxc = -1;
-    if (o.have) {
-        const long long P = a.pitch, S = a.plane;
-        const float *s = a.src;
+    if (__builtin_expect(R.g.have != 0, 1)) {
         const int yl = o.rr;
+        const long long b0 = R.g.mid.o, bm = row_cursor_ym<!DOWN>(R.g), bp = row_cursor_yp<!DOWN>(R.g);
         unsigned m0_kept;
         asm volatile("s_waitcnt lgkmcnt(0)" ::: "memory");
-        if (BC == LB_BC_PERIODIC) {
-            const int c = a.nx - 1 - x4;
-            const bool wrap_w = x4 == 0, wrap_e = c >= 0 && c < 4;
-            if (wrap_w) {
-                const float *e = s + a.nx - 1;
-                asm volatile("s_mov_b32 %0, m0\n\ts_mov_b32 m0, %4\n\ts_nop 0\n\tglobal_load_lds_dword %1, off\n\t"
-                             "s_add_u32 m0, m0, 0x100\n\ts_nop 0\n\tglobal_load_lds_dword %2, off\n\t"
-                             "s_add_u32 m0, m0, 0x100\n\ts_nop 0\n\tglobal_load_lds_dword %3, off\n\ts_mov_b32 m0, %0"
-                             : "=&s"(m0_kept)
-                             : "v"(e + 1 * S + (long long)yl * P), "v"(e + 5 * S + (long long)ym * P), "v"(e + 8 * S + (long long)yp * P),
-                               "s"(slot + 9 * 1024 + 256)
-                             : "memory", "scc");
-            }
-            if (wrap_e) {
-                asm volatile("s_mov_b32 %0, m0\n\ts_mov_b32 m0, %4\n\ts_nop 0\n\tglobal_load_lds_dword %1, off\n\t"
-                             "s_add_u32 m0, m0, 0x100\n\ts_nop 0\n\tglobal_load_lds_dword %2, off\n\t"
-                             "s_add_u32 m0, m0, 0x100\n\ts_nop 0\n\tglobal_load_lds_dword %3, off\n\ts_mov_b32 m0, %0"
-                             : "=&s"(m0_kept)
-                             : "v"(s + 3 * S + (long long)yl * P), "v"(s + 6 * S + (long long)ym * P), "v"(s + 7 * S + (long long)yp * P),
-                               "s"(slot + 9 * 1024 + 256)
-                             : "memory", "scc");
-            }
-        }
-        const u4v r0 = deep_rsrc_words(s + (long long)yl * P - 1), rm = deep_rsrc_words(s + (long long)ym * P - 1),
-                  rp = deep_rsrc_words(s + (long long)yp * P - 1);
+        const u4v r0 = deep_rsrc_words(b0), rm = deep_rsrc_words(bm), rp = deep_rsrc_words(bp);
         const unsigned S4 = (unsigned)a.plane * 4u;
         const int v0 = x4 * 4, v4 = v0 + 4, v8 = v0 + 8;
         asm volatile("s_mov_b32 %0, m0\n\ts_mov_b32 m0, %15\n\ts_nop 0\n\tbuffer_load_dwordx4 %2, %4, 0 offen lds\n\t"
@@ -252,20 +299,15 @@
     }
 }
 template <int BC, bool MASK>
-__device__ __forceinline__ void deep_row_take_lds(const f4a (*S)[64], int lane, Row1 &o)
+__device__ __forceinline__ void deep_row_take_lds(int have, const f4a (*S)[64], int lane, Row1 &o)
 {
     asm volatile("s_waitcnt vmcnt(0)" ::: "memory");
-    if (o.have) {
+    if (have) {
 #pragma unroll
         for (int k = 0; k < 9; ++k) o.q[k] = S[k][lane];
         const unsigned *X = reinterpret_cast<const unsigned *>(S[9]);
         o.mk = MASK ? __builtin_bit_cast(uc4, X[lane]) : uc4{0, 0, 0, 0};
         o.wp = WrapPatch{0.f, 0.f, 0.f, 0.f, 0.f, 0.f};
-        if (BC == LB_BC_PERIODIC) {
-            const float e1 = __builtin_bit_cast(float, X[64 + lane]), e2 = __builtin_bit_cast(float, X[128 + lane]),
-                        e3 = __builtin_bit_cast(float, X[192 + lane]);
-            o.wp = WrapPatch{e1, e2, e3, e1, e2, e3};
-        }
     } else {
         o.wp = WrapPatch{0.f, 0.f, 0.f, 0.f, 0.f, 0.f};
 #pragma unroll
@@ -274,9 +316,9 @@
     }
 }
 
-__device__ __forceinline__ void deep_row_store(const StepArgs &a, int r, int x4, const f4a (&t)[9])
-{
-    const __amdgpu_buffer_rsrc_t rd = __builtin_amdgcn_make_buffer_rsrc(deep_uniform(a.dst + (long long)r * a.pitch), 0, DEEP_NUM_RECORDS, 0x00020000);
+__device__ __forceinline__ void deep_row_store(const StepArgs &a, long long row, int x4, const f4a (&t)[9])
+{
+    const __amdgpu_buffer_rsrc_t rd = __builtin_amdgcn_make_buffer_rsrc(reinterpret_cast<float *>((unsigned long long)row), 0, DEEP_NUM_RECORDS, 0x00020000);
     const unsigned S4 = (unsigned)a.plane * 4u;
     const int vo = x4 * 4;
     asm volatile("" ::: "memory");
@@ -290,7 +332,7 @@
 }
 
 template <int BC, bool MASK, bool MACRO, int D, int RW, bool DOWN, int NST, int S, int ROLE = DEEP_WHOLE>
-__device__ __forceinline__ void deep_stage(const StepArgs &a, const DeepCtx &cx, const int i, const int it,
+__device__ __forceinline__ void deep_stage(const StepArgs &a, const DeepCtx &cx, const DeepRows &R, const int i, const int it,
                                            DeepState<RW, D - 1 - RW> &st, f4a (&qin)[9], f4a &r4, f4a &u4, f4a &v4)
 {
     if constexpr (S <= D) {
@@ -321,7 +363,7 @@
                 if (!(a.diag & (1 << 22)))
 #endif
                 if (cx.store_lane) {
-                    deep_row_store(a, r, x4, t);
+                    deep_row_store(a, R.st.o, x4, t);
                     if (MACRO) {
                         const long long m = (long long)r * a.fpitch;
                         store_moments(a, m, x4, r4, u4, v4);
@@ -332,7 +374,7 @@
                     if constexpr (S <= RW) deep_publish<DOWN>(cx.other + (D - 2 - RW) * DEEP_WSLOTS, lane, S == 1 ? 5 : 2, t);
                     else deep_publish<DOWN>(cx.other + (S - RW - 1) * DEEP_WSLOTS, lane, 2 + 3 * (S & 1), t);
                 }
-                deep_stage<BC, MASK, MACRO, D, RW, DOWN, NST, S + 1, ROLE>(a, cx, i, it, st, t, r4, u4, v4);
+                deep_stage<BC, MASK, MACRO, D, RW, DOWN, NST, S + 1, ROLE>(a, cx, R, i, it, st, t, r4, u4, v4);
             }
         } else if constexpr (NST == S - 1) {
             if constexpr (K <= RW) window_push_dir<DOWN>(st.w[K - 1], qin);
@@ -342,8 +384,8 @@
 }
 
 template <int BC, bool MASK, bool MACRO, int D, int RW, int PFD, bool DOWN, int NST, int PAR = -1, int ROLE = DEEP_WHOLE>
-__device__ __forceinline__ void deep_iter(const StepArgs &a, const DeepCtx &cx, const int i_, DeepState<RW, D - 1 - RW> &st, Row1 &cur,
-                                          Row1 &nxt)
+__device__ __forceinline__ void deep_iter(const StepArgs &a, const DeepCtx &cx, DeepRows &R, const int i_, DeepState<RW, D - 1 - RW> &st,
+                                          Row1 &cur, Row1 &nxt)
 {
     static_assert(RW >= 0 && RW <= 2 && D - 1 - RW >= 1 && (ROLE == DEEP_WHOLE ? D - 2 > RW : D - 2 >= RW),
                   "register windows hand over through the last LDS window while it is idle");
@@ -355,16 +397,28 @@
     f4a (*MB)[64] = cx.mine + (D - 2 - RW) * DEEP_WSLOTS;
     if (RW >= 1 && NST == 2) { st.w[0].g2 = MB[5][lane]; st.w[0].g5 = MB[6][lane]; st.w[0].g6 = MB[7][lane]; }
     if (RW >= 2 && NST == 3) { st.w[RW >= 2 ? 1 : 0].g2 = MB[2][lane]; st.w[RW >= 2 ? 1 : 0].g5 = MB[3][lane]; st.w[RW >= 2 ? 1 : 0].g6 = MB[4][lane]; }
+    constexpr bool MERGED = ROLE == DEEP_FRONT || (ROLE == DEEP_WHOLE && PFD && DEEP_MANUAL);
+    const int have_cur = MERGED ? R.flight : (cur.have ? 1 : 0);
 #ifdef LB_DIAG
     if (!((a.diag & (1 << 23)) && i > 0))
 #endif
     if constexpr (ROLE != DEEP_BACK) {
         if (ROLE == DEEP_FRONT) {
-            deep_row_take_lds<BC, MASK>(cx.dma, lane, cur);
-            deep_row_issue_lds<BC, MASK>(a, row_at(min(i + 1, cx.n_iter - 1)), x4, cx.dma_off, nxt);
+            row_cursor_step_to<!DOWN>(R.m, R.g, i + 1, cx.n_iter);
+            deep_row_take_lds<BC, MASK>(have_cur, cx.dma, lane, cur);
+            if (BC == LB_BC_PERIODIC && __builtin_expect(R.seam != 0, 0)) {
+                deep_seam_take_lds(a, have_cur, x4, cx.dma, lane, cur);
+                deep_seam_issue_lds<DOWN>(a, R, x4, cx.dma_off);
+            }
+            deep_row_issue_lds<BC, MASK, DOWN>(a, R, x4, cx.dma_off, nxt);
         } else if (PFD && DEEP_MANUAL) {
+            row_cursor_step_to<!DOWN>(R.m, R.g, i + 1, cx.n_iter);
             deep_row_take<BC, MASK, (NST < D ? 0 : (MACRO ? 12 : 9))>(cur);
-            deep_row_issue<BC, MASK>(a, row_at(min(i + 1, cx.n_iter - 1)), x4, nxt);
+            if (BC == LB_BC_PERIODIC && __builtin_expect(R.seam != 0, 0)) {
+                deep_seam_take(a, have_cur, x4, cur);
+                deep_seam_issue<DOWN>(a, R, x4);
+            }
+            deep_row_issue<BC, MASK, DOWN>(a, R, x4, nxt);
         } else {
             static_assert(PFD == 1 || ROLE == DEEP_BACK, "a march that gathers its rows gathers them one ahead");
             deep_row_load<BC, MASK>(a, row_at(min(i + 1, cx.n_iter - 1)), x4, nxt);
@@ -372,27 +426,32 @@
     }
     f4a (&q1)[9] = cur.q;
     f4a r4, u4, v4;
+    if (ROLE != DEEP_BACK) {
+        if (__builtin_expect(have_cur != 0, 1)) {
+            if (!MERGED) gather_merge<BC, true>(a, x4, q1, cur.wp);
+            LB_DEEP_NOCOLLIDE collide_row<BC, MASK, true>(a, x4, a.y0 + cur.rr, q1, cur.mk, r4, u4, v4);
+        } else if (ROLE == DEEP_WHOLE && PFD && DEEP_MANUAL) {
+            deep_row_none(cur);
+        }
+    }
     const uc4 mk = cur.mk;
-    if (ROLE != DEEP_BACK && cur.have) {
-        gather_merge<BC, true>(a, x4, q1, cur.wp);
-        LB_DEEP_NOCOLLIDE collide_row<BC, MASK, true>(a, x4, a.y0 + cur.rr, q1, mk, r4, u4, v4);
-    }
     if (NST == 1) {
         if constexpr (RW >= 1) deep_publish<DOWN>(cx.other + (D - 2 - RW) * DEEP_WSLOTS, lane, 5, q1);
         else deep_publish<DOWN>(cx.other, lane, 2 + 3 * 1, q1);
     }
-    deep_stage<BC, MASK, MACRO, D, RW, DOWN, NST, 2, ROLE>(a, cx, i, it, st, q1, r4, u4, v4);
+    deep_stage<BC, MASK, MACRO, D, RW, DOWN, NST, 2, ROLE>(a, cx, R, i, it, st, q1, r4, u4, v4);
+    if (NST == D && ROLE != DEEP_FRONT) R.st = row_track_next<!DOWN>(R.m, R.st);
     if (MASK) st.mhist = ((st.mhist | mask_word(mk)) << 1) & (0x01010101u * (unsigned)(((1 << D) - 2) & 0xff));
     if (ROLE == DEEP_WHOLE && NST < D) __syncthreads();
 }
 
 template <int BC, bool MASK, bool MACRO, int D, int RW, int PFD, bool DOWN, int NST>
-__device__ __forceinline__ void deep_fill(const StepArgs &a, const DeepCtx &cx, DeepState<RW, D - 1 - RW> &st, Row1 &ra, Row1 &rb)
+__device__ __forceinline__ void deep_fill(const StepArgs &a, const DeepCtx &cx, DeepRows &R, DeepState<RW, D - 1 - RW> &st, Row1 &ra, Row1 &rb)
 {
     if constexpr (NST < D) {
-        if ((NST & 1) == 0) deep_iter<BC, MASK, MACRO, D, RW, PFD, DOWN, NST>(a, cx, NST - 1, st, rb, ra);
-        else deep_iter<BC, MASK, MACRO, D, RW, PFD, DOWN, NST>(a, cx, NST - 1, st, ra, rb);
-        deep_fill<BC, MASK, MACRO, D, RW, PFD, DOWN, NST + 1>(a, cx, st, ra, rb);
+        if ((NST & 1) == 0) deep_iter<BC, MASK, MACRO, D, RW, PFD, DOWN, NST>(a, cx, R, NST - 1, st, rb, ra);
+        else deep_iter<BC, MASK, MACRO, D, RW, PFD, DOWN, NST>(a, cx, R, NST - 1, st, ra, rb);
+        deep_fill<BC, MASK, MACRO, D, RW, PFD, DOWN, NST + 1>(a, cx, R, st, ra, rb);
     }
 }
 
@@ -411,24 +470,29 @@
     auto row_at = [&](int p) { return DOWN ? ym - 1 - p : ym + p; };
     static_assert(PFD == 1, "a whole march gathers one row ahead");
     Row1 ra, rb;
-    if (DEEP_MANUAL) deep_row_issue<BC, MASK>(a, row_at(0), cx.x4, ra);
-    else deep_row_load<BC, MASK>(a, row_at(0), cx.x4, ra);
-    deep_fill<BC, MASK, MACRO, D, RW, PFD, DOWN, 1>(a, cx, st, ra, rb);
+    DeepRows R = deep_rows_begin<BC, DOWN>(a, row_at(0), cx.x4);
+    if (DEEP_MANUAL) {
+        if (BC == LB_BC_PERIODIC && R.seam) deep_seam_issue<DOWN>(a, R, cx.x4);
+        deep_row_issue<BC, MASK, DOWN>(a, R, cx.x4, ra);
+    } else {
+        deep_row_load<BC, MASK>(a, row_at(0), cx.x4, ra);
+    }
+    deep_fill<BC, MASK, MACRO, D, RW, PFD, DOWN, 1>(a, cx, R, st, ra, rb);
     if (DEEP_MANUAL) asm volatile("s_waitcnt vmcnt(0)" ::: "memory");
     if (!deep_pairs(MASK, BC)) {
         if ((D - 1) & 1) ra = rb;
         for (int i = D - 1; i < cx.n_iter; ++i) {
-            deep_iter<BC, MASK, MACRO, D, RW, PFD, DOWN, D>(a, cx, i, st, ra, rb);
+            deep_iter<BC, MASK, MACRO, D, RW, PFD, DOWN, D>(a, cx, R, i, st, ra, rb);
             ra = rb;
         }
     } else {
         constexpr int P0 = (D - 1) & 1;
         int i = D - 1;
         for (; i + 1 < cx.n_iter; i += 2) {
-            deep_iter<BC, MASK, MACRO, D, RW, PFD, DOWN, D, P0>(a, cx, i, st, P0 ? rb : ra, P0 ? ra : rb);
-            deep_iter<BC, MASK, MACRO, D, RW, PFD, DOWN, D, 1 - P0>(a, cx, i + 1, st, P0 ? ra : rb, P0 ? rb : ra);
-        }
-        if (i < cx.n_iter) deep_iter<BC, MASK, MACRO, D, RW, PFD, DOWN, D, P0>(a, cx, i, st, P0 ? rb : ra, P0 ? ra : rb);
+            deep_iter<BC, MASK, MACRO, D, RW, PFD, DOWN, D, P0>(a, cx, R, i, st, P0 ? rb : ra, P0 ? ra : rb);
+            deep_iter<BC, MASK, MACRO, D, RW, PFD, DOWN, D, 1 - P0>(a, cx, R, i + 1, st, P0 ? ra : rb, P0 ? rb : ra);
+        }
+        if (i < cx.n_iter) deep_iter<BC, MASK, MACRO, D, RW, PFD, DOWN, D, P0>(a, cx, R, i, st, P0 ? rb : ra, P0 ? ra : rb);
     }
     if (DEEP_MANUAL) asm volatile("s_waitcnt vmcnt(0)" ::: "memory");
 }
diff --git a/2d-lb_amd/csrc/kernels_deep2.h b/2d-lb_amd/csrc/kernels_deep2.h
--- a/2d-lb_amd/csrc/kernels_deep2.h
+++ b/2d-lb_amd/csrc/kernels_deep2.h
@@ -10,18 +10,18 @@
 __device__ __forceinline__ void deep2_barrier() { asm volatile("s_waitcnt lgkmcnt(0)\n\ts_barrier" ::: "memory"); }
 
 template <int BC, bool MASK, int F, int RW, bool DOWN, int NST>
-__device__ __forceinline__ void deep2_front_fill(const StepArgs &a, const DeepCtx &cx, DeepState<RW, F - 1 - RW> &st, Row1 &ra, Row1 &rb,
-                                                 int &trip)
+__device__ __forceinline__ void deep2_front_fill(const StepArgs &a, const DeepCtx &cx, DeepRows &R, DeepState<RW, F - 1 - RW> &st, Row1 &ra,
+                                                 Row1 &rb, int &trip)
 {
     if constexpr (NST < F) {
         deep2_barrier();
         if (trip < cx.n_iter) {
-            if ((NST & 1) == 0) deep_iter<BC, MASK, false, F, RW, 1, DOWN, NST, -1, DEEP_FRONT>(a, cx, NST - 1, st, rb, ra);
-            else deep_iter<BC, MASK, false, F, RW, 1, DOWN, NST, -1, DEEP_FRONT>(a, cx, NST - 1, st, ra, rb);
+            if ((NST & 1) == 0) deep_iter<BC, MASK, false, F, RW, 1, DOWN, NST, -1, DEEP_FRONT>(a, cx, R, NST - 1, st, rb, ra);
+            else deep_iter<BC, MASK, false, F, RW, 1, DOWN, NST, -1, DEEP_FRONT>(a, cx, R, NST - 1, st, ra, rb);
         }
         deep2_barrier();
         ++trip;
-        deep2_front_fill<BC, MASK, F, RW, DOWN, NST + 1>(a, cx, st, ra, rb, trip);
+        deep2_front_fill<BC, MASK, F, RW, DOWN, NST + 1>(a, cx, R, st, ra, rb, trip);
     }
 }
 
@@ -40,9 +40,11 @@
     DeepState<RW, F - 1 - RW> st = {};
     auto row_at = [&](int p) { return DOWN ? ym - 1 - p : ym + p; };
     Row1 ra, rb;
-    deep_row_issue_lds<BC, MASK>(a, row_at(0), cx.x4, cx.dma_off, ra);
+    DeepRows R = deep_rows_begin<BC, DOWN>(a, row_at(0), cx.x4);
+    if (BC == LB_BC_PERIODIC && R.seam) deep_seam_issue_lds<DOWN>(a, R, cx.x4, cx.dma_off);
+    deep_row_issue_lds<BC, MASK, DOWN>(a, R, cx.x4, cx.dma_off, ra);
     int trip = 0;
-    deep2_front_fill<BC, MASK, F, RW, DOWN, 1>(a, cx, st, ra, rb, trip);
+    deep2_front_fill<BC, MASK, F, RW, DOWN, 1>(a, cx, R, st, ra, rb, trip);
     if ((F - 1) & 1) ra = rb;
     for (; trip < trips; ++trip) {
 #ifdef LB_DIAG
@@ -50,7 +52,7 @@
 #endif
         deep2_barrier();
         if (trip < cx.n_iter) {
-            deep_iter<BC, MASK, false, F, RW, 1, DOWN, F, -1, DEEP_FRONT>(a, cx, trip, st, ra, rb);
+            deep_iter<BC, MASK, false, F, RW, 1, DOWN, F, -1, DEEP_FRONT>(a, cx, R, trip, st, ra, rb);
             ra = rb;
         }
 #ifdef LB_DIAG
@@ -72,15 +74,16 @@
 }
 
 template <int BC, bool MASK, bool MACRO, int DB, int RW, bool DOWN, int NST>
-__device__ __forceinline__ void deep2_back_fill(const StepArgs &a, const DeepCtx &cx, DeepState<RW, DB - 1 - RW> &st, Row1 &cur, int &j)
+__device__ __forceinline__ void deep2_back_fill(const StepArgs &a, const DeepCtx &cx, DeepRows &R, DeepState<RW, DB - 1 - RW> &st, Row1 &cur,
+                                                int &j)
 {
     if constexpr (NST < DB) {
         if (j < cx.n_iter) deep2_take<MASK>(cx, cur);
         deep2_barrier();
-        if (j < cx.n_iter) deep_iter<BC, MASK, MACRO, DB, RW, 0, DOWN, NST, -1, DEEP_BACK>(a, cx, NST - 1, st, cur, cur);
+        if (j < cx.n_iter) deep_iter<BC, MASK, MACRO, DB, RW, 0, DOWN, NST, -1, DEEP_BACK>(a, cx, R, NST - 1, st, cur, cur);
         deep2_barrier();
         ++j;
-        deep2_back_fill<BC, MASK, MACRO, DB, RW, DOWN, NST + 1>(a, cx, st, cur, j);
+        deep2_back_fill<BC, MASK, MACRO, DB, RW, DOWN, NST + 1>(a, cx, R, st, cur, j);
     }
 }
 
@@ -104,15 +107,16 @@
         deep2_barrier();
         deep2_barrier();
     }
+    DeepRows R = deep_rows_begin<BC, DOWN>(a, DOWN ? ym - 1 : ym, cx.x4);
     int j = 0;
-    deep2_back_fill<BC, MASK, MACRO, DB, RW, DOWN, 1>(a, cx, st, cur, j);
+    deep2_back_fill<BC, MASK, MACRO, DB, RW, DOWN, 1>(a, cx, R, st, cur, j);
     for (; j + F < trips; ++j) {
         if (j < cx.n_iter) deep2_take<MASK>(cx, cur);
 #ifdef LB_DIAG
         if (!(a.diag & (1 << 24)))
 #endif
         deep2_barrier();
-        if (j < cx.n_iter) deep_iter<BC, MASK, MACRO, DB, RW, 0, DOWN, DB, -1, DEEP_BACK>(a, cx, j, st, cur, cur);
+        if (j < cx.n_iter) deep_iter<BC, MASK, MACRO, DB, RW, 0, DOWN, DB, -1, DEEP_BACK>(a, cx, R, j, st, cur, cur);
 #ifdef LB_DIAG
         if (!(a.diag & (1 << 24)))
 #endif
diff --git a/2d-lb_amd/csrc/kernels_fused.h b/2d-lb_amd/csrc/kernels_fused.h
--- a/2d-lb_amd/csrc/kernels_fused.h
+++ b/2d-lb_amd/csrc/kernels_fused.h
@@ -2,6 +2,7 @@
 #include <type_traits>
 #include "d2q9_cell.h"
 #include "plan_consts.h"
+#include "row_cursor.h"
 
 struct StepArgs {
     const float *src;
@@ -385,13 +386,7 @@
 
 __device__ __forceinline__ bool step1_rows(const StepArgs &a, int r, int &rr, int &ym, int &yp)
 {
-    const int h = a.h, w = a.wrap_y, per = h - (w == 2 ? 1 : 0);
-    const int wr = r < 0 ? r + per : (r >= h ? r - per : r);
-    rr = w ? wr : r;
-    const int m = rr - 1, p = rr + 1;
-    ym = (w && m < 0) ? h - w : m;
-    yp = (w && p >= h) ? w - 1 : p;
-    return w || (r < 0 ? a.ghost_s != 0 : (r >= h ? a.ghost_n != 0 : true));
+    return step1_rows_of(a.h, a.wrap_y, a.ghost_s, a.ghost_n, r, rr, ym, yp);
 }
 
 template <int BC, bool MASK>
diff --git a/2d-lb_amd/csrc/row_cursor.h b/2d-lb_amd/csrc/row_cursor.h
--- /dev/null
+++ b/2d-lb_amd/csrc/row_cursor.h
@@ -0,0 +1,91 @@
+#pragma once
+
+#if defined(__HIPCC__)
+#define LB_ROW_FN __host__ __device__ __forceinline__
+#else
+#define LB_ROW_FN inline
+#endif
+
+LB_ROW_FN bool step1_rows_of(int h, int wrap_y, int ghost_s, int ghost_n, int r, int &rr, int &ym, int &yp)
+{
+    const int w = wrap_y, per = h - (w == 2 ? 1 : 0);
+    const int wr = r < 0 ? r + per : (r >= h ? r - per : r);
+    rr = w ? wr : r;
+    const int m = rr - 1, p = rr + 1;
+    ym = (w && m < 0) ? h - w : m;
+    yp = (w && p >= h) ? w - 1 : p;
+    return w || (r < 0 ? ghost_s != 0 : (r >= h ? ghost_n != 0 : true));
+}
+
+struct RowMarch {
+    int h, wrap_y, ghost_s, ghost_n;
+    unsigned pitch_b;
+    long long span_b;
+};
+LB_ROW_FN RowMarch row_march(int h, int wrap_y, int ghost_s, int ghost_n, unsigned pitch_bytes)
+{
+    return RowMarch{h, wrap_y, ghost_s, ghost_n, pitch_bytes, (long long)(h - 1) * (long long)pitch_bytes};
+}
+
+template <bool UP>
+LB_ROW_FN int row_next(const RowMarch &m, int y, long long &by)
+{
+    if (UP) {
+        const bool wrap = m.wrap_y && y + 1 >= m.h;
+        by = wrap ? -m.span_b : (long long)m.pitch_b;
+        return wrap ? m.wrap_y - 1 : y + 1;
+    }
+    const bool wrap = m.wrap_y && y - 1 < 0;
+    by = wrap ? m.span_b : -(long long)m.pitch_b;
+    return wrap ? m.h - m.wrap_y : y - 1;
+}
+
+struct RowTrack {
+    int y;
+    long long o;
+};
+template <bool UP>
+LB_ROW_FN RowTrack row_track_next(const RowMarch &m, const RowTrack &t)
+{
+    long long by;
+    const int y = row_next<UP>(m, t.y, by);
+    return RowTrack{y, t.o + by};
+}
+
+struct RowCursor {
+    int have;
+    RowTrack mid;
+    long long lag, lead;
+    LB_ROW_FN int rr() const { return mid.y; }
+};
+template <bool UP> LB_ROW_FN long long row_cursor_ym(const RowCursor &c) { return UP ? c.lag : c.lead; }
+template <bool UP> LB_ROW_FN long long row_cursor_yp(const RowCursor &c) { return UP ? c.lead : c.lag; }
+
+template <bool UP>
+LB_ROW_FN RowCursor row_cursor_begin(const RowMarch &m, int r0, long long base)
+{
+    int rr, ym, yp;
+    RowCursor c;
+    (void)step1_rows_of(m.h, m.wrap_y, m.ghost_s, m.ghost_n, r0, rr, ym, yp);
+    c.have = m.wrap_y | (r0 < 0 ? m.ghost_s : (r0 >= m.h ? m.ghost_n : 1));
+    c.mid = RowTrack{rr, base + (long long)rr * (long long)m.pitch_b};
+    c.lag = base + (long long)(UP ? ym : yp) * (long long)m.pitch_b;
+    c.lead = base + (long long)(UP ? yp : ym) * (long long)m.pitch_b;
+    return c;
+}
+template <bool UP>
+LB_ROW_FN void row_cursor_step(const RowMarch &m, RowCursor &c)
+{
+    long long by;
+    const int y = row_next<UP>(m, c.mid.y, by);
+    c.lag = c.mid.o;
+    c.mid = RowTrack{y, c.lead};
+    (void)row_next<UP>(m, y, by);
+    c.lead += by;
+    c.have = m.wrap_y | (y < 0 ? m.ghost_s : (y >= m.h ? m.ghost_n : 1));
+}
+template <bool UP>
+LB_ROW_FN void row_cursor_step_to(const RowMarch &m, RowCursor &c, int pos, int n_pos)
+{
+    if (pos < n_pos) row_cursor_step<UP>(m, c);
+}
```

Measured after the change: 485,500. No clear change (-0.0%).
